# HKUDS/GPT-ST

Measured on AMD Instinct MI355X. Metric: pretrain steps/sec at (B=32,T=12,N=170,C=64), higher is better.
Workload: dtype f32; 1 GPU; BASELINE configs[1]: PEMS08-shape synthetic pretrain step, per-GPU B=32 T=12 N=170 C=64 base=1, epoch 200/300 (adaptive mask + KL), fwd+loss+bwd+clip+Adam, hipGraph=True, 4 full optimiser steps on 4 different resident batches per graph replay; global_batch=32, parallelism=dp1

## Files before the change

### gpt-st_amd/csrc/apply.hip

```cpp
#include "mfma_tile.h"
#include "wgrad64.h"
#include "kl_guest.h"
#ifdef GPTST_DEBUG
__device__ long long g_ap_ts[64];
static thread_local int g_ap_dbg = 0;
extern "C" int gptst_ap_dbg(int v) { g_ap_dbg = v; return 0; }
extern "C" int gptst_ap_ts(long long* out) { return (int)hipMemcpyFromSymbol(out, HIP_SYMBOL(g_ap_ts), sizeof(long long) * 64); }
#else
static constexpr int g_ap_dbg = 0;
#endif
thread_local int g_apply_tpw = 0;
thread_local int g_apply128_minwg = 768;
thread_local int g_apply128_v1 = 0;

template <int C, int PRO, int EPI>
__global__ __launch_bounds__(256) void apply_kernel(const float* __restrict__ A, const float* __restrict__ A2,
                                                    const float* __restrict__ W, long w_gstride, int transw,
                                                    const float* __restrict__ bias, const float* __restrict__ resid,
                                                    const float* __restrict__ resid2, float* __restrict__ out, float* __restrict__ colsum, RowMap rm, int dbg) {
    using T = Tile<C>;
    int tsi = 0;
#ifdef GPTST_DEBUG
#define TS() do { if (dbg && blockIdx.x == 100 && blockIdx.y == 0 && threadIdx.x == 0) g_ap_ts[tsi] = clock64(); ++tsi; } while (0)
#else
// ... 183 lines not shown
#pragma unroll
        for (int ct = 0; ct < 4; ++ct) acc[ct] = (f32x4){0.f, 0.f, 0.f, 0.f};
#pragma unroll
        for (int q = 0; q < 4; ++q) {
            const float av[4] = {a[q].x, a[q].y, a[q].z, a[q].w};
#pragma unroll
            for (int e = 0; e < 4; ++e) {
                acc[0] = __builtin_amdgcn_mfma_f32_16x16x4f32(av[e], bv[q][e].x, acc[0], 0, 0, 0);
                acc[1] = __builtin_amdgcn_mfma_f32_16x16x4f32(av[e], bv[q][e].y, acc[1], 0, 0, 0);
                acc[2] = __builtin_amdgcn_mfma_f32_16x16x4f32(av[e], bv[q][e].z, acc[2], 0, 0, 0);
                acc[3] = __builtin_amdgcn_mfma_f32_16x16x4f32(av[e], bv[q][e].w, acc[3], 0, 0, 0);
            }
        }
        SB();
#pragma unroll
        for (int r = 0; r < 4; ++r) {
            if (t * 16 + kk * 4 + r < rm.M) {
                float4 y = f4add(make_float4(acc[0][r], acc[1][r], acc[2][r], acc[3][r]), bias4);
                if (EPI == EPI_RES_LRELU) {
                    y = f4add(y, rv[r]);
                    y.x = lrelu(y.x); y.y = lrelu(y.y); y.z = lrelu(y.z); y.w = lrelu(y.w);
                }
                if (EPI == EPI_LRELU) { y.x = lrelu(y.x); y.y = lrelu(y.y); y.z = lrelu(y.z); y.w = lrelu(y.w); }
                if (EPI == EPI_ADD_DPRE) {
                    const float4 d = rv[r], o = rv2[r];
                    y.x = fmaf(d.x, lrelu_grad_from_out(o.x), y.x); y.y = fmaf(d.y, lrelu_grad_from_out(o.y), y.y);
                    y.z = fmaf(d.z, lrelu_grad_from_out(o.z), y.z); y.w = fmaf(d.w, lrelu_grad_from_out(o.w), y.w);
                }
                st4(out + orow[r], y);
            }
        }
    }
    if (colsum != nullptr) {
#pragma unroll
        for (int q = 0; q < 4; ++q) {
            cs[q].x = group_sum<16>(cs[q].x); cs[q].y = group_sum<16>(cs[q].y);
            cs[q].z = group_sum<16>(cs[q].z); cs[q].w = group_sum<16>(cs[q].w);
            if (j == 0) st4(&csl[wave][16 * q + 4 * kk], cs[q]);
        }
        __syncthreads();
        if (wave == 0) colsum[((size_t)blockIdx.y * rm.G + g) * C + lane] = (csl[0][lane] + csl[1][lane]) + (csl[2][lane] + csl[3][lane]);
    }
}

static void apply64_geometry(const RowMap& rm, bool has_colsum, int& tpw, int& gy) {
    const int ntiles = (rm.M + 15) / 16;
    long tot = (long)rm.G * ntiles;
    tpw = (int)((tot + 4 * 512 - 1) / (4 * 512));
    if (tpw > 2) tpw = 2;
    if (has_colsum && rm.G == 1) { const int lim = (ntiles + 4 * 128 - 1) / (4 * 128); if (tpw < lim) tpw = lim; }
    if (g_apply_tpw > 0) tpw = g_apply_tpw;
    if (tpw < 1) tpw = 1;
    gy = (ntiles + 4 * tpw - 1) / (4 * tpw);
}

template <int PRO, int EPI>
static void launch_apply64_t(const float* A, const float* A2, const float* W, long gs, int transw, const float* bias, const float* resid,
                             const float* resid2, float* out, float* colsum, RowMap rm, hipStream_t st) {
    int tpw, gy;
    apply64_geometry(rm, colsum != nullptr, tpw, gy);
    hipLaunchKernelGGL((apply64_kernel<PRO, EPI>), dim3(rm.G, gy), dim3(256), 0, st, A, A2, W, gs, transw, bias, resid, resid2, out, colsum, rm, tpw);
}

static int launch_apply64(const float* A, const float* A2, const float* W, long gs, int transw, const float* bias, const float* resid,
                          const float* resid2, float* out, float* colsum, RowMap rm, int pro, int epi, hipStream_t st) {
    if (pro == PRO_NONE && epi == EPI_PLAIN) launch_apply64_t<PRO_NONE, EPI_PLAIN>(A, A2, W, gs, transw, bias, resid, resid2, out, colsum, rm, st);
    else if (pro == PRO_NONE && epi == EPI_RES_LRELU) launch_apply64_t<PRO_NONE, EPI_RES_LRELU>(A, A2, W, gs, transw, bias, resid, resid2, out, colsum, rm, st);
    else if (pro == PRO_DPRE && epi == EPI_PLAIN) launch_apply64_t<PRO_DPRE, EPI_PLAIN>(A, A2, W, gs, transw, bias, resid, resid2, out, colsum, rm, st);
    else if (pro == PRO_NONE && epi == EPI_ADD_DPRE) launch_apply64_t<PRO_NONE, EPI_ADD_DPRE>(A, A2, W, gs, transw, bias, resid, resid2, out, colsum, rm, st);
    else if (pro == PRO_NONE && epi == EPI_LRELU) launch_apply64_t<PRO_NONE, EPI_LRELU>(A, A2, W, gs, transw, bias, resid, resid2, out, colsum, rm, st);
    else return GPTST_EARG;
    GPTST_CHECK_LAUNCH();
    return GPTST_OK;
}

template <int PRO, int U>
__global__ __launch_bounds__(256, 2) void wgrad64_kernel(const float* __restrict__ A, const float* __restrict__ D,
                                                         const float* __restrict__ D2, float* __restrict__ dW, RowMap rm,
                                                         int rows_per_split, int ostride, int csa) {
    __shared__ __attribute__((aligned(16))) float smem[WGRAD64_SMEM_FLOATS];
    wgrad64_body<PRO, U>(A, D, D2, dW, rm, rows_per_split, ostride, csa, blockIdx.x, blockIdx.y, smem);
}

template <int KIND, int CHAIN>
__global__ __launch_bounds__(256, 2) void applywg64_kernel(const float* __restrict__ dOut, const float* __restrict__ Y,
                                                            const float* __restrict__ S, const float* __restrict__ W, long w_gstride,
                                                            const float* __restrict__ resid, const float* __restrict__ resid2,
                                                            float* __restrict__ dS, float* __restrict__ dW, float* __restrict__ colsum,
                                                            RowMap rm, int tiles_per_wave) {
    __shared__ __attribute__((aligned(16))) float lds[APPLYWG64_LDS_FLOATS];
    applywg64_body<KIND, CHAIN>(dOut, Y, S, W, w_gstride, resid, resid2, dS, dW, colsum, rm, tiles_per_wave, blockIdx.x, blockIdx.y, lds);
}

GPTST_INTERNAL int gptst_apply_wgrad_geometry(int mode, int BT, int N, int* tpw) {
    RowMap rm = make_rowmap(mode, BT, N);
    int gy;
    apply64_geometry(rm, false, *tpw, gy);
    return gy;
}

extern "C" int gptst_apply_wgrad_nsplit(int mode, int BT, int N) {
    RowMap rm = make_rowmap(mode, BT, N);
    int tpw, gy;
    apply64_geometry(rm, false, tpw, gy);
    return gy;
}

extern "C" int gptst_apply_wgrad(const float* dOut, const float* Y, const float* S, const float* W, float* dS, float* dW, float* colsum,
                                 int premul, int mode, int BT, int N, int C, void* stream) {
    if (!dOut || !S || !W || !dS || !dW || BT <= 0 || N <= 0 || mode < 0 || mode > 1 || (Y && premul)) return GPTST_EARG;
    if (C != 64) return GPTST_ESHAPE;
    RowMap rm = make_rowmap(mode, BT, N);
    int tpw, gy;
    apply64_geometry(rm, false, tpw, gy);
    const dim3 grid(rm.G, gy);
    hipStream_t st = (hipStream_t)stream;
    if (Y) hipLaunchKernelGGL((applywg64_kernel<0, 0>), grid, dim3(256), 0, st, dOut, Y, S, W, (long)C * C, nullptr, nullptr, dS, dW, colsum, rm, tpw);
    else if (!premul) hipLaunchKernelGGL((applywg64_kernel<0, 1>), grid, dim3(256), 0, st, dOut, Y, S, W, (long)C * C, nullptr, nullptr, dS, dW, colsum, rm, tpw);
    else hipLaunchKernelGGL((applywg64_kernel<0, 2>), grid, dim3(256), 0, st, dOut, Y, S, W, (long)C * C, nullptr, nullptr, dS, dW, colsum, rm, tpw);
    GPTST_CHECK_LAUNCH();
    return GPTST_OK;
}

extern "C" int gptst_linear_bwd_nsplit(int rows) {
    RowMap rm = make_rowmap(2, rows, 1);
    int tpw, gy;
    apply64_geometry(rm, false, tpw, gy);
    return gy;
}

extern "C" int gptst_linear_bwd(const float* dY, const float* X, const float* Wp, const float* dOut, const float* out, float* dX, float* dWp,
                                float* dbp, int premul, int rows, int C, void* stream) {
    if (!dY || !X || !Wp || !dOut || !dX || !dWp || !dbp || rows <= 0 || (out && premul)) return GPTST_EARG;
    if (C != 64) return GPTST_ESHAPE;
    RowMap rm = make_rowmap(2, rows, 1);
    int tpw, gy;
    apply64_geometry(rm, false, tpw, gy);
    hipStream_t st = (hipStream_t)stream;
    if (out) hipLaunchKernelGGL((applywg64_kernel<1, 0>), dim3(1, gy), dim3(256), 0, st, dY, nullptr, X, Wp, 0L, dOut, out, dX, dWp, dbp, rm, tpw);
    else if (!premul) hipLaunchKernelGGL((applywg64_kernel<1, 1>), dim3(1, gy), dim3(256), 0, st, dY, nullptr, X, Wp, 0L, dOut, nullptr, dX, dWp, dbp, rm, tpw);
    else hipLaunchKernelGGL((applywg64_kernel<1, 2>), dim3(1, gy), dim3(256), 0, st, dY, nullptr, X, Wp, 0L, dOut, X, dX, dWp, dbp, rm, tpw);
    GPTST_CHECK_LAUNCH();
    return GPTST_OK;
}

template <int C, int PRO>
__global__ __launch_bounds__(256) void wgrad_kernel(const float* __restrict__ A, const float* __restrict__ D,
                                                    const float* __restrict__ D2, float* __restrict__ dW,
                                                    RowMap rm, int rows_per_split) {
    constexpr int NCT = C / 32;
    constexpr int TPW = NCT * NCT / 4;
    const int lane = threadIdx.x & 63, wave = threadIdx.x >> 6;
    const int j = lane & 31, h = lane >> 5;
    const int g = blockIdx.x, sp = blockIdx.y;
    const int mbeg = sp * rows_per_split;
    const int mend = min(rm.M, mbeg + rows_per_split);
    const int it = (wave * TPW) / NCT;
    f32x16 acc[TPW];
#pragma unroll
    for (int u = 0; u < TPW; ++u)
#pragma unroll
        for (int r = 0; r < 16; ++r) acc[u][r] = 0.f;

    for (int m = mbeg + h; m < mend + h; m += 2) {
        float a = 0.f;
        float d[TPW];
#pragma unroll
        for (int u = 0; u < TPW; ++u) d[u] = 0.f;
        if (m < mend) {
            const size_t off = ((size_t)g * rm.rs_g + (size_t)m * rm.rs_m) * C;
            a = A[off + it * 32 + j];
#pragma unroll
            for (int u = 0; u < TPW; ++u) {
                const int jt = (wave * TPW + u) % NCT;
                float dv = D[off + jt * 32 + j];
                if (PRO == PRO_DPRE) dv *= lrelu_grad_from_out(D2[off + jt * 32 + j]);
                d[u] = dv;
            }
        }
#pragma unroll
        for (int u = 0; u < TPW; ++u) acc[u] = __builtin_amdgcn_mfma_f32_32x32x2f32(a, d[u], acc[u], 0, 0, 0);
    }
    float* o = dW + ((size_t)sp * rm.G + g) * C * C;
#pragma unroll
    for (int u = 0; u < TPW; ++u) {
        const int jt = (wave * TPW + u) % NCT;
#pragma unroll
        for (int r = 0; r < 16; ++r) {
            const int row = (r & 3) + 8 * (r >> 2) + 4 * h;
            o[(size_t)(it * 32 + row) * C + jt * 32 + j] = acc[u][r];
        }
    }
}

#define AP128_NW 8
template <int PRO, int EPI, bool CS>
__global__ __launch_bounds__(64 * AP128_NW, 4) void apply128_kernel(const float* __restrict__ A, const float* __restrict__ A2,
                                                                    const float* __restrict__ W, long w_gstride, int transw,
                                                                    const float* __restrict__ bias, const float* __restrict__ resid,
                                                                    const float* __restrict__ resid2, float* __restrict__ out,
                                                                    float* __restrict__ colsum, RowMap rm, int tiles_per_wave) {
    constexpr int C = 128, Q = C / 16;
    extern __shared__ __attribute__((aligned(16))) float smem[];
    float* Wl = smem;
    float* csl = smem + C * C;
    const int lane = threadIdx.x & 63, wave = threadIdx.x >> 6;
    const int j = lane & 15, kk = lane >> 4;
    const int g = blockIdx.x;
    const int ntiles = (rm.M + 15) / 16;
    const int t0 = (blockIdx.y * AP128_NW + wave) * tiles_per_wave, t1 = min(ntiles, t0 + tiles_per_wave);
    float4 bias0 = f4zero(), bias1 = f4zero();
    if (bias != nullptr) { bias0 = ld4(bias + (size_t)g * C + 4 * j); bias1 = ld4(bias + (size_t)g * C + 64 + 4 * j); }
    float4 a[Q], on[Q];
    auto fetch = [&](int t) {
        const int m = min(t * 16 + j, rm.M - 1);
        const size_t off = ((size_t)g * rm.rs_g + (size_t)m * rm.rs_m) * C + 4 * kk;
#pragma unroll
        for (int q = 0; q < Q; ++q) {
            a[q] = ld4(A + off + 16 * q);
            if (PRO == PRO_DPRE) on[q] = ld4(A2 + off + 16 * q);
        }
    };
    if (t0 < t1) fetch(t0);
    load_w_lds<C, 64 * AP128_NW>(Wl, W + (size_t)g * w_gstride, transw, threadIdx.x);
// ... 346 lines not shown
```

### gpt-st_amd/csrc/guidein.hip

```cpp
#include "mfma_tile.h"
#include "kl_guest.h"

#define GI_CHUNKS 3

template <int C>
__global__ __launch_bounds__(256) void guide_in_fwd_kernel(const float* __restrict__ src, int lda, const float* __restrict__ w1,
                                                           const float* __restrict__ b1, const float* __restrict__ Wn, const float* __restrict__ bn,
                                                           float* __restrict__ h1, int BT, int N) {
    constexpr int LPR = C / 4, RPP = 256 / LPR, NQ = 256 / C, U = 4;
    __shared__ __attribute__((aligned(16))) float part[NQ * 2 * C];
    __shared__ __attribute__((aligned(16))) float vec[2 * C];
    const int n = blockIdx.x, chunk = blockIdx.y, tid = threadIdx.x;
    {
        const int q = tid / C, o = tid % C;
        const float* W = Wn + (size_t)n * C * C;
        float au = 0.f, ac = 0.f;
#pragma unroll 8
        for (int i = q * (C / NQ); i < (q + 1) * (C / NQ); ++i) {
            const float x = W[(size_t)i * C + o];
            au = fmaf(w1[i], x, au);
            ac = fmaf(b1[i], x, ac);
        }
        part[(q * 2 + 0) * C + o] = au;
        part[(q * 2 + 1) * C + o] = ac;
// ... 2 lines not shown
    if (tid < C) {
        float s0 = 0.f, s1 = 0.f;
#pragma unroll
        for (int q = 0; q < NQ; ++q) { s0 += part[(q * 2 + 0) * C + tid]; s1 += part[(q * 2 + 1) * C + tid]; }
        vec[tid] = s0; vec[C + tid] = s1 + bn[(size_t)n * C + tid];
    }
    __syncthreads();
    const int slot = tid / LPR, c4 = tid % LPR;
    const float4 u4 = ld4(vec + 4 * c4), k4 = ld4(vec + C + 4 * c4);
    const int per = (BT + GI_CHUNKS - 1) / GI_CHUNKS, r0 = chunk * per, r1 = min(BT, r0 + per);
    for (int rr = r0 + slot; rr < r1; rr += RPP * U) {
        float s[U];
#pragma unroll
        for (int u = 0; u < U; ++u) s[u] = src[((size_t)min(rr + u * RPP, r1 - 1) * N + n) * lda];
#pragma unroll
        for (int u = 0; u < U; ++u) {
            const int r = rr + u * RPP;
            if (r < r1) {
                float4 y = f4fma(s[u], u4, k4);
                y.x = lrelu(y.x); y.y = lrelu(y.y); y.z = lrelu(y.z); y.w = lrelu(y.w);
                st4(h1 + ((size_t)r * N + n) * C + 4 * c4, y);
            }
        }
    }
}

template <int C>
__global__ __launch_bounds__(256) void guide_in_bwd_kernel(const float* __restrict__ dPre, const float* __restrict__ src, int lda,
                                                           const float* __restrict__ w1, const float* __restrict__ b1, const float* __restrict__ Wn,
                                                           float* __restrict__ dWb, float* __restrict__ dinp, int BT, int N) {
    __shared__ __attribute__((aligned(16))) float lds[guide_in_bwd_lds_floats<C>()];
    guide_in_bwd_body<C>(dPre, src, lda, w1, b1, Wn, dWb, dinp, BT, N, blockIdx.x, lds);
}

extern "C" int gptst_guide_in_fwd(const float* src, int lda, const float* w1, const float* b1, const float* Wn, const float* bn, float* h1,
                                  int BT, int N, int C, void* stream) {
    if (!src || !w1 || !b1 || !Wn || !bn || !h1 || BT <= 0 || N <= 0 || lda <= 0) return GPTST_EARG;
    if (C == 64) hipLaunchKernelGGL((guide_in_fwd_kernel<64>), dim3(N, GI_CHUNKS), dim3(256), 0, (hipStream_t)stream, src, lda, w1, b1, Wn, bn, h1, BT, N);
    else if (C == 128) hipLaunchKernelGGL((guide_in_fwd_kernel<128>), dim3(N, GI_CHUNKS), dim3(256), 0, (hipStream_t)stream, src, lda, w1, b1, Wn, bn, h1, BT, N);
    else return GPTST_ESHAPE;
    GPTST_CHECK_LAUNCH();
    return GPTST_OK;
}

extern "C" int gptst_guide_in_bwd(const float* dPre, const float* src, int lda, const float* w1, const float* b1, const float* Wn, float* dWb,
                                  float* dinp, int BT, int N, int C, void* stream) {
    if (!dPre || !src || !w1 || !b1 || !Wn || !dWb || !dinp || BT <= 0 || N <= 0 || lda <= 0) return GPTST_EARG;
    if (C == 64) hipLaunchKernelGGL((guide_in_bwd_kernel<64>), dim3(N), dim3(256), 0, (hipStream_t)stream, dPre, src, lda, w1, b1, Wn, dWb, dinp, BT, N);
    else if (C == 128) hipLaunchKernelGGL((guide_in_bwd_kernel<128>), dim3(N), dim3(256), 0, (hipStream_t)stream, dPre, src, lda, w1, b1, Wn, dWb, dinp, BT, N);
    else return GPTST_ESHAPE;
    GPTST_CHECK_LAUNCH();
    return GPTST_OK;
}

template <int C>
__global__ __launch_bounds__(256) void guide_uc_kernel(const float* __restrict__ w1, const float* __restrict__ b1, const float* __restrict__ Wn,
                                                       const float* __restrict__ bn, float* __restrict__ uc) {
    constexpr int NQ = 256 / C;
    __shared__ __attribute__((aligned(16))) float part[NQ * 2 * C];
    const int n = blockIdx.x, tid = threadIdx.x;
    const int q = tid / C, o = tid % C;
    const float* W = Wn + (size_t)n * C * C;
    float au = 0.f, ac = 0.f;
#pragma unroll 8
    for (int i = q * (C / NQ); i < (q + 1) * (C / NQ); ++i) {
        const float x = W[(size_t)i * C + o];
        au = fmaf(w1[i], x, au);
        ac = fmaf(b1[i], x, ac);
    }
    part[(q * 2 + 0) * C + o] = au;
    part[(q * 2 + 1) * C + o] = ac;
    __syncthreads();
    if (tid < C) {
        float s0 = 0.f, s1 = 0.f;
#pragma unroll
        for (int qq = 0; qq < NQ; ++qq) { s0 += part[(qq * 2 + 0) * C + tid]; s1 += part[(qq * 2 + 1) * C + tid]; }
        uc[(size_t)n * 2 * C + tid] = s0;
        uc[(size_t)n * 2 * C + C + tid] = s1 + bn[(size_t)n * C + tid];
    }
}

#define GH_P 68
extern thread_local int g_apply_tpw;
__global__ __launch_bounds__(256, 2) void guide_head_fwd_kernel(const float* __restrict__ src, int lda, const float* __restrict__ uc,
                                                                const float* __restrict__ Wbt, const float* __restrict__ bbt,
                                                                const float* __restrict__ W3, const float* __restrict__ b3,
                                                                float* __restrict__ h1, float* __restrict__ h2, float* __restrict__ prob,
                                                                int* __restrict__ label, int N, int J, int tiles_per_wave) {
    constexpr int C = 64;
    __shared__ __attribute__((aligned(16))) float Wl[C * C];
    __shared__ __attribute__((aligned(16))) float tl[4][16 * GH_P];
    const int lane = threadIdx.x & 63, wave = threadIdx.x >> 6;
    const int j = lane & 15, kk = lane >> 4;
    const int g = blockIdx.x;
    const int ntiles = (N + 15) / 16;
    const int t0 = (blockIdx.y * 4 + wave) * tiles_per_wave, t1 = min(ntiles, t0 + tiles_per_wave);
    const float4 bias4 = ld4(bbt + (size_t)g * C + 4 * j);
    float4 bw[4];
#pragma unroll
    for (int q = 0; q < 4; ++q) bw[q] = j < J ? ld4(W3 + (size_t)j * C + 16 * q + 4 * kk) : f4zero();
    const float bj = j < J ? b3[j] : 0.f;
    float sn;
    float4 un[4], cn[4];
    auto fetch = [&](int t) {
        const int m = min(t * 16 + j, N - 1);
        sn = src[((size_t)g * N + m) * lda];
#pragma unroll
        for (int q = 0; q < 4; ++q) { un[q] = ld4(uc + (size_t)m * 2 * C + 16 * q + 4 * kk); cn[q] = ld4(uc + (size_t)m * 2 * C + C + 16 * q + 4 * kk); }
    };
    if (t0 < t1) fetch(t0);
    load_w_lds<C, 256>(Wl, Wbt + (size_t)g * C * C, 0, threadIdx.x);
    __syncthreads();
    float4 bv[4][4];
#pragma unroll
    for (int q = 0; q < 4; ++q)
#pragma unroll
        for (int e = 0; e < 4; ++e) bv[q][e] = ld4(Wl + (16 * q + 4 * kk + e) * C + 4 * j);
    float* tile = tl[wave];
    for (int t = t0; t < t1; ++t) {
        float4 a[4];
        const int mrow = t * 16 + j;
#pragma unroll
        for (int q = 0; q < 4; ++q) {
            float4 y = f4fma(sn, un[q], cn[q]);
            y.x = lrelu(y.x); y.y = lrelu(y.y); y.z = lrelu(y.z); y.w = lrelu(y.w);
            if (mrow < N) st4(h1 + ((size_t)g * N + mrow) * C + 16 * q + 4 * kk, y); else y = f4zero();
            a[q] = y;
        }
        if (t + 1 < t1) fetch(t + 1);
        SB();
        f32x4 acc[4];
#pragma unroll
        for (int ct = 0; ct < 4; ++ct) acc[ct] = (f32x4){0.f, 0.f, 0.f, 0.f};
#pragma unroll
        for (int q = 0; q < 4; ++q) {
            const float av[4] = {a[q].x, a[q].y, a[q].z, a[q].w};
#pragma unroll
            for (int e = 0; e < 4; ++e) {
                acc[0] = __builtin_amdgcn_mfma_f32_16x16x4f32(av[e], bv[q][e].x, acc[0], 0, 0, 0);
                acc[1] = __builtin_amdgcn_mfma_f32_16x16x4f32(av[e], bv[q][e].y, acc[1], 0, 0, 0);
                acc[2] = __builtin_amdgcn_mfma_f32_16x16x4f32(av[e], bv[q][e].z, acc[2], 0, 0, 0);
                acc[3] = __builtin_amdgcn_mfma_f32_16x16x4f32(av[e], bv[q][e].w, acc[3], 0, 0, 0);
            }
        }
        SB();
#pragma unroll
        for (int r = 0; r < 4; ++r) {
            const int m = t * 16 + kk * 4 + r;
            float4 y = f4add(make_float4(acc[0][r], acc[1][r], acc[2][r], acc[3][r]), bias4);
            y.x = lrelu(y.x); y.y = lrelu(y.y); y.z = lrelu(y.z); y.w = lrelu(y.w);
            if (m < N) st4(h2 + ((size_t)g * N + m) * C + 4 * j, y);
            st4(tile + (kk * 4 + r) * GH_P + 4 * j, y);
        }
        f32x4 z0 = {0.f, 0.f, 0.f, 0.f}, z1 = {0.f, 0.f, 0.f, 0.f};
#pragma unroll
        for (int q = 0; q < 4; ++q) {
            const float4 x = ld4(tile + j * GH_P + 16 * q + 4 * kk);
            z0 = __builtin_amdgcn_mfma_f32_16x16x4f32(x.x, bw[q].x, z0, 0, 0, 0);
            z1 = __builtin_amdgcn_mfma_f32_16x16x4f32(x.y, bw[q].y, z1, 0, 0, 0);
            z0 = __builtin_amdgcn_mfma_f32_16x16x4f32(x.z, bw[q].z, z0, 0, 0, 0);
            z1 = __builtin_amdgcn_mfma_f32_16x16x4f32(x.w, bw[q].w, z1, 0, 0, 0);
        }
#pragma unroll
        for (int r = 0; r < 4; ++r) {
            const int m = t * 16 + kk * 4 + r;
            const size_t i = (size_t)g * N + m;
            float v = z0[r] + z1[r] + bj;
            const float mx = group_max<16>(j < J ? v : -3.0e38f);
            const float e = j < J ? expf(v - mx) : 0.f;
            v = e / group_sum<16>(e);
            if (m < N && j < J) prob[i * J + j] = v;
            const float vv = j < J ? v : -3.0e38f;
            const float gm = group_max<16>(vv);
            const int first = (int)(-group_max<16>(vv == gm ? -(float)j : -3.0e38f));
            if (m < N && j == 0) label[i] = first;
        }
    }
}

extern "C" int gptst_guide_uc_floats(int N, int C) { return N * 2 * C; }

extern "C" int gptst_guide_head_fwd(const float* src, int lda, const float* w1, const float* b1, const float* Wn, const float* bn, const float* Wbt,
                                    const float* bbt, const float* W3, const float* b3, float* uc, float* h1, float* h2, float* prob, int* label,
                                    int BT, int N, int C, int J, void* stream) {
    if (!src || !w1 || !b1 || !Wn || !bn || !Wbt || !bbt || !W3 || !b3 || !uc || !h1 || !h2 || !prob || !label || BT <= 0 || N <= 0 || lda <= 0 || J <= 0)
        return GPTST_EARG;
    if (C != 64 || J > 16) return GPTST_ESHAPE;
    hipLaunchKernelGGL((guide_uc_kernel<64>), dim3(N), dim3(256), 0, (hipStream_t)stream, w1, b1, Wn, bn, uc);
    const int ntiles = (N + 15) / 16;
    int tpw = 1;
    if (g_apply_tpw > 0) tpw = g_apply_tpw;
    if (tpw < 1) tpw = 1;
    const int gy = (ntiles + 4 * tpw - 1) / (4 * tpw);
    hipLaunchKernelGGL(guide_head_fwd_kernel, dim3(BT, gy), dim3(256), 0, (hipStream_t)stream, src, lda, uc, Wbt, bbt, W3, b3, h1, h2, prob, label, N, J, tpw);
    GPTST_CHECK_LAUNCH();
    return GPTST_OK;
}
```

### gpt-st_amd/csrc/hypertem.hip

```cpp
#include "mfma_tile.h"
#include "wgrad64.h"
#include "kl_guest.h"
GPTST_STAMP_TABLES(hypertem)
GPTST_HANDOFF_COUNTER(hypertem)

#define HT_T 12
#ifndef HT_OCC
#define HT_OCC 2
#endif
#ifdef GPTST_DEBUG
__device__ long long g_ht_ts[64];
static thread_local int g_ht_dbg = 0, g_ht_nt_override = 0;
extern "C" int gptst_ht_dbg(int v) { g_ht_dbg = v; return 0; }
extern "C" int gptst_ht_variant(int fwd, int bwd) { g_ht_nt_override = fwd; (void)bwd; return 0; }
extern "C" int gptst_ht_ts(long long* out) { return (int)hipMemcpyFromSymbol(out, HIP_SYMBOL(g_ht_ts), sizeof(long long) * 64); }
#define HT_DBG(d) (d)
#else
#define HT_DBG(d) 0
static constexpr int g_ht_dbg = 0, g_ht_nt_override = 0;
#endif

__device__ __forceinline__ bool ht_work_at(int L, int ntiles, int B, int& b, int& tile) {
    const int xcd = L & 7, slot = L >> 3;
    b = xcd + 8 * (slot / ntiles);
    tile = slot % ntiles;
    return b < B;
}
__device__ __forceinline__ bool ht_work(int ntiles, int B, int& b, int& tile) { return ht_work_at(blockIdx.x, ntiles, B, b, tile); }

static int ht_pick_nt(int B, int N) {
    if (g_ht_nt_override >= 4 && g_ht_nt_override <= 16) return g_ht_nt_override;
    (void)B; (void)N;
    return 16;
}

__global__ __launch_bounds__(256, HT_OCC) void hypertem_fwd_kernel(const float* __restrict__ X, const float* __restrict__ G,
                                                              const float* __restrict__ Wbt, const float* __restrict__ bbt,
                                                              float* __restrict__ R_out, float* __restrict__ out, int N, int B, int NT,
                                                              int dbg) {
    constexpr int C = 64, P = C + 4, GP = 145;
    int tsi = 0;
#ifdef GPTST_DEBUG
#define TS() do { if ((dbg & 1) && blockIdx.x == 59 && threadIdx.x == 0) g_ht_ts[tsi] = clock64(); ++tsi; } while (0)
#else
#define TS() __builtin_amdgcn_sched_barrier(0)
#endif
    TS();
    extern __shared__ __attribute__((aligned(16))) float smem[];
    float* Xs = smem;
    float* Gs = Xs + HT_T * NT * P;
    int b, tile;
    if (!ht_work((N + NT - 1) / NT, B, b, tile)) return;
    const int n0 = tile * NT;
    const int tid = threadIdx.x, lane = tid & 63, wave = tid >> 6;
    {
        const int nl = tid >> 4, c4 = tid & 15;
        const int n = min(n0 + nl, N - 1);
        float4 v[HT_T];
        float gv[9];
#pragma unroll
        for (int t = 0; t < HT_T; ++t) v[t] = ld4(X + (((size_t)b * HT_T + t) * N + n) * C + 4 * c4);
#pragma unroll
        for (int k = 0; k < 9; ++k) gv[k] = G[min(n0 * 144 + tid + k * 256, N * 144 - 1)];
        if (nl < NT) {
#pragma unroll
            for (int t = 0; t < HT_T; ++t) st4(Xs + (t * NT + nl) * P + 4 * c4, n0 + nl < N ? v[t] : f4zero());
        }
#pragma unroll
        for (int k = 0; k < 9; ++k) {
            const int i = tid + k * 256;
            if (i < NT * 144) Gs[(i / 144) * GP + i % 144] = (n0 + i / 144 < N) ? gv[k] : 0.f;
        }
    }
    __syncthreads();
    TS();
    const int j = lane & 15, kk = lane >> 4;
    const int ja = j < NT ? j : 0;
    float4 bv[C / 16][4];
    float4 b4;
#define HT_LOAD_W(tt) do {                                                                                         \
        const float* W_ = Wbt + ((size_t)b * HT_T + (tt)) * C * C;                                                 \
        _Pragma("unroll") for (int q = 0; q < C / 16; ++q)                                                         \
            _Pragma("unroll") for (int e = 0; e < 4; ++e) bv[q][e] = ld4(W_ + (size_t)(16 * q + 4 * kk + e) * C + 4 * j); \
        b4 = ld4(bbt + ((size_t)b * HT_T + (tt)) * C + 4 * j);                                                     \
    } while (0)
    HT_LOAD_W(wave);
    for (int t = wave; t < HT_T; t += 4) {
        const size_t g = (size_t)b * HT_T + t;
        TS();
        float4 a4[C / 16];
#pragma unroll
        for (int q = 0; q < C / 16; ++q) a4[q] = f4zero();
        {
            const float* gr = Gs + ja * GP + t * HT_T;
            const float* xr = Xs + ja * P + 4 * kk;
#pragma unroll
            for (int u = 0; u < HT_T; ++u) {
                const float gu = gr[u];
#pragma unroll
                for (int q = 0; q < C / 16; ++q) a4[q] = f4fma(gu, ld4(xr + u * NT * P + 16 * q), a4[q]);
            }
        }
        TS();
        f32x4 acc[C / 16];
#pragma unroll
        for (int ct = 0; ct < C / 16; ++ct) acc[ct] = (f32x4){0.f, 0.f, 0.f, 0.f};
#pragma unroll
        for (int q = 0; q < C / 16; ++q) {
            const float av[4] = {a4[q].x, a4[q].y, a4[q].z, a4[q].w};
#pragma unroll
            for (int e = 0; e < 4; ++e) {
                acc[0] = __builtin_amdgcn_mfma_f32_16x16x4f32(av[e], bv[q][e].x, acc[0], 0, 0, 0);
                acc[1] = __builtin_amdgcn_mfma_f32_16x16x4f32(av[e], bv[q][e].y, acc[1], 0, 0, 0);
                acc[2] = __builtin_amdgcn_mfma_f32_16x16x4f32(av[e], bv[q][e].z, acc[2], 0, 0, 0);
                acc[3] = __builtin_amdgcn_mfma_f32_16x16x4f32(av[e], bv[q][e].w, acc[3], 0, 0, 0);
            }
        }
        TS();
        const float4 bias = b4;
        if (t + 4 < HT_T) HT_LOAD_W(t + 4);
        TS();
        if (R_out != nullptr && j < NT && n0 + j < N) {
#pragma unroll
            for (int q = 0; q < C / 16; ++q) st4_far(R_out + (g * N + n0 + j) * C + 16 * q + 4 * kk, a4[q]);
        }
#pragma unroll
        for (int r = 0; r < 4; ++r) {
            const int nl = kk * 4 + r;
            if (nl < NT && n0 + nl < N) {
                float4 y = f4add(f4add(make_float4(acc[0][r], acc[1][r], acc[2][r], acc[3][r]), bias), ld4(Xs + (t * NT + nl) * P + 4 * j));
                y.x = lrelu(y.x); y.y = lrelu(y.y); y.z = lrelu(y.z); y.w = lrelu(y.w);
                st4(out + (g * N + n0 + nl) * C + 4 * j, y);
            }
        }
        TS();
    }
}

static size_t ht_smem(int NT) { return ((size_t)HT_T * NT * 68 + NT * 145) * sizeof(float); }

extern "C" int gptst_hypertem_fwd(const float* X, const float* G, const float* Wbt, const float* bbt, float* R_out, float* out, int B,
                                  int T, int N, int C, void* stream) {
    if (!X || !G || !Wbt || !bbt || !out || T != HT_T) return GPTST_EARG;
    if (C != 64) return GPTST_ESHAPE;
    static int done = 0;
    if (!done) { hipFuncSetAttribute((const void*)hypertem_fwd_kernel, hipFuncAttributeMaxDynamicSharedMemorySize, (int)ht_smem(16)); done = 1; }
    const int NT = ht_pick_nt(B, N);
    hipLaunchKernelGGL(hypertem_fwd_kernel, dim3(8 * ((B + 7) / 8) * ((N + NT - 1) / NT)), dim3(256), ht_smem(NT), (hipStream_t)stream, X, G, Wbt, bbt, R_out, out, N, B, NT, g_ht_dbg);
    GPTST_CHECK_LAUNCH();
    return GPTST_OK;
}

template <bool HASY, bool PREMUL, int PAIR>
__device__ __forceinline__ void hypertem_bwd_stage(const float* __restrict__ dOut, const float* __restrict__ Y,
                                                   const float* __restrict__ X, const float* __restrict__ G,
                                                   const float* __restrict__ Wbt, float* __restrict__ dX,
                                                   float* __restrict__ dbias, float* __restrict__ dG, int N, int B, int dbg, int b, int tile,
                                                   float* __restrict__ smem, float4 (&dp)[HT_T]) {
    constexpr int C = 64, P = C + 4, GP = 145, NT = 16;
    float* Ds = smem;
    float* Gs = Ds + HT_T * NT * P;
    const int n0 = tile * NT;
    const int tid = threadIdx.x, lane = tid & 63, wave = tid >> 6;
    const int nl = tid >> 4, c4 = tid & 15;
    const bool valid = n0 + nl < N;
    const size_t rowoff = ((size_t)b * HT_T * N + min(n0 + nl, N - 1)) * C + 4 * c4;
    const int j = lane & 15, kk = lane >> 4;
    float4 aq[C / 16][C / 16];
#define HT_LOAD_WT(tt) do {                                                                                         \
        const float* W_ = Wbt + ((size_t)b * HT_T + (tt)) * C * C;                                                  \
        _Pragma("unroll") for (int it = 0; it < C / 16; ++it)                                                       \
            _Pragma("unroll") for (int q = 0; q < C / 16; ++q) aq[it][q] = ld4(W_ + (size_t)(it * 16 + j) * C + 16 * q + 4 * kk); \
    } while (0)
    static_assert(!(HASY && PREMUL), "one sign operand per launch");
    const float* __restrict__ Sg = HASY ? Y : X;
    float4 yv[HT_T];
    float gv[9];
    unsigned sb0 = 0u, sb1 = 0u;
#pragma unroll
    for (int t = 0; t < 4; ++t) { if (PAIR != 2) dp[t] = ld4(dOut + rowoff + (size_t)t * N * C); if (HASY || PREMUL) yv[t] = ld4(Sg + rowoff + (size_t)t * N * C); }
#pragma unroll
    for (int k = 0; k < 9; ++k) gv[k] = G[min(n0 * 144 + tid + k * 256, N * 144 - 1)];
    HT_LOAD_WT(wave);
#pragma unroll
    for (int t = 4; t < HT_T; ++t) { if (PAIR != 2) dp[t] = ld4(dOut + rowoff + (size_t)t * N * C); if (HASY || PREMUL) yv[t] = ld4(Sg + rowoff + (size_t)t * N * C); }
    SB();
#pragma unroll
    for (int grp = 0; grp < HT_T / 4; ++grp) {
#pragma unroll
        for (int tt = 0; tt < 4; ++tt) {
            const int t = 4 * grp + tt;
            float4 v = dp[t];
            if (HASY) v = make_float4(dp[t].x * lrelu_grad_from_out(yv[t].x), dp[t].y * lrelu_grad_from_out(yv[t].y),
                                      dp[t].z * lrelu_grad_from_out(yv[t].z), dp[t].w * lrelu_grad_from_out(yv[t].w));
            if (PREMUL) {
                const unsigned m4 = (yv[t].x > 0.f ? 1u : 0u) | (yv[t].y > 0.f ? 2u : 0u) | (yv[t].z > 0.f ? 4u : 0u) | (yv[t].w > 0.f ? 8u : 0u);
                if (t < 8) sb0 |= m4 << (4 * t); else sb1 |= m4 << (4 * (t - 8));
            }
            if (!valid) v = f4zero();
            dp[t] = v;
            st4(Ds + (t * NT + nl) * P + 4 * c4, v);
        }
        if (grp == 0) {
#pragma unroll
            for (int k = 0; k < 9; ++k) {
                const int i = tid + k * 256;
                Gs[(i / 144) * GP + i % 144] = (n0 + i / 144 < N) ? gv[k] : 0.f;
            }
        }
        __syncthreads();
        SB();
        if (PAIR != 0 && grp == 0) GPTST_STAMP(PAIR == 2 ? 6 : 1);
        const int t = 4 * grp + wave;
        if (HT_DBG(dbg) & 32) continue;
        const size_t g = (size_t)b * HT_T + t;
        float* dt = Ds + t * NT * P;
        float s = 0.f;
        if (dbias != nullptr) {
#pragma unroll
            for (int r = 0; r < NT; ++r) s += dt[r * P + lane];
        }
        float4 bq[C / 16];
#pragma unroll
        for (int q = 0; q < C / 16; ++q) bq[q] = ld4(dt + j * P + 16 * q + 4 * kk);
        f32x4 acc[C / 16];
#pragma unroll
        for (int it = 0; it < C / 16; ++it) acc[it] = (f32x4){0.f, 0.f, 0.f, 0.f};
        if (!(HT_DBG(dbg) & 64))
#pragma unroll
        for (int q = 0; q < C / 16; ++q) {
#pragma unroll
// ... 483 lines not shown
                const float4 bias = b4;
                if (t + NW < HT_T) HTC_LOAD_W(S.Wbt, S.bbt, t + NW);
                SB();
                if (S.R_out != nullptr && n0 + j < N) {
#pragma unroll
                    for (int q = 0; q < C / 16; ++q) st4_far(S.R_out + (g * N + n0 + j) * C + 16 * q + 4 * kk, a4[q]);
                }
#pragma unroll
                for (int r = 0; r < 4; ++r) {
                    const int nl = kk * 4 + r;
                    if (n0 + nl < N) {
                        float4 y = f4add(f4add(make_float4(acc[0][r], acc[1][r], acc[2][r], acc[3][r]), bias), ld4(Xs + (t * NT + nl) * P + 4 * j));
                        y.x = lrelu(y.x); y.y = lrelu(y.y); y.z = lrelu(y.z); y.w = lrelu(y.w);
                        st4(S.out + (g * N + n0 + nl) * C + 4 * j, y);
                    }
                }
            }
        }
    }
#undef HTC_LOAD_G
#undef HTC_STORE_G
#undef HTC_LOAD_W
}

static int ht_chain_args(HtChain& ch, const float* X, int nstage, const void* Gs, const void* Wbts, const void* bbts, const void* Rs, const void* outs,
                         int B, int T, int N, int C) {
    if (!X || nstage < 1 || nstage > 3 || !Gs || !Wbts || !bbts || !Rs || !outs || T != HT_T || B <= 0 || N <= 0) return GPTST_EARG;
    if (C != 64) return GPTST_ESHAPE;
    ch.nstage = nstage; ch.X = X;
    for (int s = 0; s < 3; ++s) {
        const int k = s < nstage ? s : nstage - 1;
        ch.st[s] = HtStage{((const float* const*)Gs)[k], ((const float* const*)Wbts)[k], ((const float* const*)bbts)[k],
                           ((float* const*)Rs)[k], ((float* const*)outs)[k]};
        if (!ch.st[s].G || !ch.st[s].Wbt || !ch.st[s].bbt || !ch.st[s].out) return GPTST_EARG;
    }
    return GPTST_OK;
}

static int ht_chain_grid(int B, int N) { return 8 * ((B + 7) / 8) * ((N + 15) / 16); }

extern "C" int gptst_hypertem_chain_fwd(const float* X, int nstage, const void* Gs, const void* Wbts, const void* bbts, const void* Rs,
                                        const void* outs, int B, int T, int N, int C, void* stream) {
    HtChain ch;
    const int rc = ht_chain_args(ch, X, nstage, Gs, Wbts, bbts, Rs, outs, B, T, N, C);
    if (rc != GPTST_OK) return rc;
    const dim3 grid(ht_chain_grid(B, N));
    const int smem = (int)ht_smem(16);
    hipStream_t st = (hipStream_t)stream;
    const KlGuest none{};
#define HTC_LAUNCH(NS_) do {                                                                                                          \
        static int done_ = 0;                                                                                                          \
        if (!done_) { (void)hipFuncSetAttribute((const void*)hypertem_chain_fwd_kernel<NS_, 0>, hipFuncAttributeMaxDynamicSharedMemorySize, smem); done_ = 1; } \
        hipLaunchKernelGGL((hypertem_chain_fwd_kernel<NS_, 0>), grid, dim3(64 * HTC_NW), smem, st, ch, N, B, none);                          \
    } while (0)
    if (nstage == 1) HTC_LAUNCH(1); else if (nstage == 2) HTC_LAUNCH(2); else HTC_LAUNCH(3);
#undef HTC_LAUNCH
    GPTST_CHECK_LAUNCH();
    return GPTST_OK;
}

GPTST_INTERNAL int gptst_tail_geometry(int rows, int* rows_per_block);
GPTST_INTERNAL int gptst_apply_wgrad_geometry(int mode, int BT, int N, int* tpw);

extern "C" int gptst_kl_guest_blocks(int stage, int B, int T, int N) {
    if (B <= 0 || T <= 0 || N <= 0) return GPTST_EARG;
    int aux;
    if (stage == 1) return gptst_tail_geometry(B * T * N, &aux);
    if (stage == 2) return B * T * gptst_apply_wgrad_geometry(0, B * T, N, &aux);
    if (stage == 3) return N;
    return GPTST_EARG;
}

extern "C" int gptst_hypertem_chain_fwd_kl(const float* X, int nstage, const void* Gs, const void* Wbts, const void* bbts, const void* Rs,
                                           const void* outs, int B, int T, int N, int C, int stage, const void* ops, int v0, int v1, int HS,
                                           int lda, float w, void* stream) {
    HtChain ch;
    const int rc = ht_chain_args(ch, X, nstage, Gs, Wbts, bbts, Rs, outs, B, T, N, C);
    if (rc != GPTST_OK) return rc;
    if (!ops || stage < 1 || stage > 3) return GPTST_EARG;
    if (nstage != 2 || HTC_NW != 4 || HS <= 0 || HS > TL_MAXJ) return GPTST_ESHAPE;
    const int nv = gptst_kl_guest_blocks(stage, B, T, N);
    if (v0 < 0 || v1 <= v0 || v1 > nv) return GPTST_EARG;
    const float* const* p = (const float* const*)ops;
    const int np = stage == 1 ? 7 : stage == 2 ? 6 : 7;
    for (int i = 0; i < np; ++i) if (!p[i]) return GPTST_EARG;
    KlGuest kg{};
    kg.base = ht_chain_grid(B, N);
    kg.v0 = v0;
    if (stage == 1) {
        TailArgs& t = kg.tail;
        t.X = p[0]; t.W = p[1]; t.prob = p[2]; t.c = p[3]; t.dX = (float*)p[4]; t.part = (float*)p[5]; t.sws = (float*)p[6];
        t.rows = B * T * N; t.J = HS; t.N = N; t.w = w; t.premul = 1;
        gptst_tail_geometry(t.rows, &t.rows_per_block);
    } else if (stage == 2) {
        kg.dOut = p[0]; kg.S = p[1]; kg.W = p[2]; kg.dS = (float*)p[3]; kg.dW = (float*)p[4]; kg.colsum = (float*)p[5];
        kg.rm = make_rowmap(0, B * T, N);
        gptst_apply_wgrad_geometry(0, B * T, N, &kg.tpw);
    } else {
        if (lda <= 0) return GPTST_EARG;
        kg.dPre = p[0]; kg.src = p[1]; kg.lda = lda; kg.w1 = p[2]; kg.b1 = p[3]; kg.Wn = p[4]; kg.dWb = (float*)p[5]; kg.dinp = (float*)p[6];
        kg.BT = B * T; kg.N = N;
    }
    const dim3 grid(kg.base + (v1 - v0));
    const size_t sg = kl_guest_lds_bytes(stage), sh = ht_smem(16);
    const int smem = (int)(sg > sh ? sg : sh);
    hipStream_t st = (hipStream_t)stream;
#define HTC_LAUNCH(G_) do {                                                                                                           \
        static int done_ = 0;                                                                                                          \
        if (!done_) { (void)hipFuncSetAttribute((const void*)hypertem_chain_fwd_kernel<2, G_>, hipFuncAttributeMaxDynamicSharedMemorySize, smem); done_ = 1; } \
        hipLaunchKernelGGL((hypertem_chain_fwd_kernel<2, G_>), grid, dim3(64 * HTC_NW), smem, st, ch, N, B, kg);                           \
    } while (0)
    if (stage == 1) HTC_LAUNCH(1); else if (stage == 2) HTC_LAUNCH(2); else HTC_LAUNCH(3);
#undef HTC_LAUNCH
    GPTST_CHECK_LAUNCH();
    return GPTST_OK;
}
```

### gpt-st_amd/csrc/kl_guest.h

```cpp
#pragma once
#include "mfma_tile.h"
#include "wgrad64.h"

#define TL_MAXJ 16

struct TailArgs {
    const float* X; const float* W; const float* b; float* dX; float* part; float* sws;
    int rows, J, rows_per_block;
    const float* src; const float* mask; float* out; int lda; float sigma, mu, thresh;
    const float* prob; const float* c; int N; float w;
    int premul;
};

template <int C>
constexpr int tail_mfma_lds_floats() { return 4 * (16 * C + 16) + 4 * 16 * 17 + 8; }

template <int KIND, int C>
__device__ __forceinline__ void tail_mfma_body(const TailArgs& t, int blk, float* __restrict__ lds) {
    constexpr int Q = C / 16, HF = C / 64;
    float (*fold)[16 * C + 16] = reinterpret_cast<float (*)[16 * C + 16]>(lds);
    float (*at)[16][17] = reinterpret_cast<float (*)[16][17]>(lds + 4 * (16 * C + 16));
    float (*reds)[4] = reinterpret_cast<float (*)[4]>(lds + 4 * (16 * C + 16) + 4 * 16 * 17);
    const int J = t.J;
    const int lane = threadIdx.x & 63, wave = threadIdx.x >> 6;
// ... 60 lines not shown
                        a[r] = (d > 0.f ? 1.f : (d < 0.f ? -1.f : 0.f)) * M * t.sigma;
                    }
                    t.out[e] = o;
                }
            }
        } else {
#pragma unroll
            for (int r = 0; r < 4; ++r) {
                const size_t i = tb + 4 * kk + r;
                const bool ok = i < r1 && j < J;
                float e_ = 0.f, p_ = 1.f;
                if (ok) { e_ = o0[r]; p_ = o1[r]; }
                const float se = group_sum<16>(e_);
                if (ok && e_ > 0.f) s0 += e_ * (logf(e_) - logf(p_));
                a[r] = ok ? t.w * (p_ * se - e_) : 0.f;
            }
        }
#pragma unroll
        for (int r = 0; r < 4; ++r) {
            gb += a[r];
#pragma unroll
            for (int hf = 0; hf < HF; ++hf) {
                gw[hf][0] = __builtin_amdgcn_mfma_f32_16x16x4f32(a[r], xd[hf][r].x, gw[hf][0], 0, 0, 0);
                gw[hf][1] = __builtin_amdgcn_mfma_f32_16x16x4f32(a[r], xd[hf][r].y, gw[hf][1], 0, 0, 0);
                gw[hf][2] = __builtin_amdgcn_mfma_f32_16x16x4f32(a[r], xd[hf][r].z, gw[hf][2], 0, 0, 0);
                gw[hf][3] = __builtin_amdgcn_mfma_f32_16x16x4f32(a[r], xd[hf][r].w, gw[hf][3], 0, 0, 0);
            }
        }
#pragma unroll
        for (int r = 0; r < 4; ++r) at[wave][4 * kk + r][j] = a[r];
        f32x4 dx[HF][4];
#pragma unroll
        for (int hf = 0; hf < HF; ++hf)
#pragma unroll
            for (int ct = 0; ct < 4; ++ct) dx[hf][ct] = (f32x4){0.f, 0.f, 0.f, 0.f};
#pragma unroll
        for (int s = 0; s < 4; ++s) {
            if (s < nks) {
                const float as = at[wave][j][4 * s + kk];
#pragma unroll
                for (int hf = 0; hf < HF; ++hf) {
                    dx[hf][0] = __builtin_amdgcn_mfma_f32_16x16x4f32(as, bd[hf][s].x, dx[hf][0], 0, 0, 0);
                    dx[hf][1] = __builtin_amdgcn_mfma_f32_16x16x4f32(as, bd[hf][s].y, dx[hf][1], 0, 0, 0);
                    dx[hf][2] = __builtin_amdgcn_mfma_f32_16x16x4f32(as, bd[hf][s].z, dx[hf][2], 0, 0, 0);
                    dx[hf][3] = __builtin_amdgcn_mfma_f32_16x16x4f32(as, bd[hf][s].w, dx[hf][3], 0, 0, 0);
                }
            }
        }
#pragma unroll
        for (int r = 0; r < 4; ++r) {
            const size_t i = tb + 4 * kk + r;
#pragma unroll
            for (int hf = 0; hf < HF; ++hf) {
                float4 v = make_float4(dx[hf][0][r], dx[hf][1][r], dx[hf][2][r], dx[hf][3][r]);
                if (t.premul) {
                    v.x *= lrelu_grad_from_out(xd[hf][r].x); v.y *= lrelu_grad_from_out(xd[hf][r].y);
                    v.z *= lrelu_grad_from_out(xd[hf][r].z); v.w *= lrelu_grad_from_out(xd[hf][r].w);
                }
                if (i < r1) st4(t.dX + i * C + 64 * hf + 4 * j, v);
            }
        }
    }
#pragma unroll
    for (int r = 0; r < 4; ++r)
#pragma unroll
        for (int hf = 0; hf < HF; ++hf) st4(&fold[wave][(4 * kk + r) * C + 64 * hf + 4 * j], make_float4(gw[hf][0][r], gw[hf][1][r], gw[hf][2][r], gw[hf][3][r]));
    gb += __shfl_xor(gb, 16, 64); gb += __shfl_xor(gb, 32, 64);
    if (kk == 0) fold[wave][16 * C + j] = gb;
    s0 = group_sum<64>(s0); s1 = group_sum<64>(s1);
    if (lane == 0) { reds[0][wave] = s0; reds[1][wave] = s1; }
    __syncthreads();
    float* mine = t.part + (size_t)blk * (J * C + J);
    for (int o = threadIdx.x; o < J * C; o += 256) mine[o] = (fold[0][o] + fold[1][o]) + (fold[2][o] + fold[3][o]);
    if ((int)threadIdx.x < J) mine[J * C + threadIdx.x] = (fold[0][16 * C + threadIdx.x] + fold[1][16 * C + threadIdx.x]) + (fold[2][16 * C + threadIdx.x] + fold[3][16 * C + threadIdx.x]);
    if (threadIdx.x == 0) {
        float* w = t.sws + 4 * (size_t)blk;
        const float v0 = (reds[0][0] + reds[0][1]) + (reds[0][2] + reds[0][3]), v1 = (reds[1][0] + reds[1][1]) + (reds[1][2] + reds[1][3]);
        if (KIND == 0) { w[0] = v0; w[1] = v1; } else { w[2] = v0; }
    }
}

constexpr int APPLYWG64_LDS_FLOATS = 4 * 64 * 64 + 4 * 64;

template <int KIND, int CHAIN>
__device__ __forceinline__ void applywg64_body(const float* __restrict__ dOut, const float* __restrict__ Y, const float* __restrict__ S,
                                               const float* __restrict__ W, long w_gstride, const float* __restrict__ resid,
                                               const float* __restrict__ resid2, float* __restrict__ dS, float* __restrict__ dW,
                                               float* __restrict__ colsum, RowMap rm, int tiles_per_wave, int g, int split, float* __restrict__ lds) {
    constexpr int C = 64, TP = C + 4;
    float* smem = lds;
    float (*csl)[C] = reinterpret_cast<float (*)[C]>(lds + 4 * C * C);
    float* Wl = smem;
    const int lane = threadIdx.x & 63, wave = threadIdx.x >> 6;
    float* tile = smem + C * C + wave * 16 * TP;
    const int j = lane & 15, kk = lane >> 4;
    const int ntiles = (rm.M + 15) / 16;
    const int t0 = (split * 4 + wave) * tiles_per_wave, t1 = min(ntiles, t0 + tiles_per_wave);
    float4 d[4], y[4], a[4];
    auto fetch = [&](int t) {
#pragma unroll
        for (int s4 = 0; s4 < 4; ++s4) {
            const int m = min(t * 16 + 4 * s4 + kk, rm.M - 1);
            const size_t off = ((size_t)g * rm.rs_g + (size_t)m * rm.rs_m) * C + 4 * j;
            d[s4] = ld4(dOut + off); a[s4] = ld4(S + off);
            if (KIND == 0 && CHAIN == 0) y[s4] = ld4(Y + off);
        }
    };
    if (t0 < t1) fetch(t0);
    load_w_lds<C, 256>(Wl, W + (size_t)g * w_gstride, KIND == 0 ? 1 : 0, threadIdx.x);
    __syncthreads();
    float4 bv[4][4];
#pragma unroll
    for (int q = 0; q < 4; ++q)
#pragma unroll
        for (int e = 0; e < 4; ++e) bv[q][e] = ld4(Wl + (16 * q + 4 * kk + e) * C + 4 * j);
    f32x4 accw[4][4];
#pragma unroll
    for (int ca = 0; ca < 4; ++ca)
#pragma unroll
        for (int cb = 0; cb < 4; ++cb) accw[ca][cb] = (f32x4){0.f, 0.f, 0.f, 0.f};
    float4 cs = f4zero();
    for (int t = t0; t < t1; ++t) {
        if (KIND == 1 && t != t0) fetch(t);
        SB();
#pragma unroll
        for (int s4 = 0; s4 < 4; ++s4) {
            float4 v = d[s4];
            if (KIND == 0 && CHAIN == 0) v = make_float4(d[s4].x * lrelu_grad_from_out(y[s4].x), d[s4].y * lrelu_grad_from_out(y[s4].y),
                                                         d[s4].z * lrelu_grad_from_out(y[s4].z), d[s4].w * lrelu_grad_from_out(y[s4].w));
            if (t * 16 + 4 * s4 + kk >= rm.M) v = f4zero();
            d[s4] = v;
            cs = f4add(cs, v);
            st4(tile + (4 * s4 + kk) * TP + 4 * j, v);
        }
#pragma unroll
        for (int s4 = 0; s4 < 4; ++s4) {
            const float sv[4] = {a[s4].x, a[s4].y, a[s4].z, a[s4].w}, dv[4] = {d[s4].x, d[s4].y, d[s4].z, d[s4].w};
#pragma unroll
            for (int ca = 0; ca < 4; ++ca)
#pragma unroll
                for (int cb = 0; cb < 4; ++cb)
                    accw[ca][cb] = __builtin_amdgcn_mfma_f32_16x16x4f32(KIND == 0 ? sv[ca] : dv[ca], KIND == 0 ? dv[cb] : sv[cb], accw[ca][cb], 0, 0, 0);
        }
        SB();
        float4 ap[4];
#pragma unroll
        for (int q = 0; q < 4; ++q) ap[q] = ld4(tile + j * TP + 16 * q + 4 * kk);
        const int tcur = t;
        if (KIND == 0 && t + 1 < t1) fetch(t + 1);
        float4 rv[4], rv2[4];
        if (KIND == 1 || CHAIN == 2) {
#pragma unroll
            for (int r = 0; r < 4; ++r) {
                const int m = min(tcur * 16 + kk * 4 + r, rm.M - 1);
                const size_t off = ((size_t)g * rm.rs_g + (size_t)m * rm.rs_m) * C + 4 * j;
                if (KIND == 1) rv[r] = ld4(resid + off);
                if (KIND == 1 && CHAIN != 1) rv2[r] = ld4(resid2 + off);
                if (KIND == 0 && CHAIN == 2) rv2[r] = ld4(S + off);
            }
        }
        SB();
        f32x4 acc[4];
#pragma unroll
        for (int ct = 0; ct < 4; ++ct) acc[ct] = (f32x4){0.f, 0.f, 0.f, 0.f};
#pragma unroll
        for (int q = 0; q < 4; ++q) {
            const float av[4] = {ap[q].x, ap[q].y, ap[q].z, ap[q].w};
#pragma unroll
            for (int e = 0; e < 4; ++e) {
                acc[0] = __builtin_amdgcn_mfma_f32_16x16x4f32(av[e], bv[q][e].x, acc[0], 0, 0, 0);
                acc[1] = __builtin_amdgcn_mfma_f32_16x16x4f32(av[e], bv[q][e].y, acc[1], 0, 0, 0);
                acc[2] = __builtin_amdgcn_mfma_f32_16x16x4f32(av[e], bv[q][e].z, acc[2], 0, 0, 0);
                acc[3] = __builtin_amdgcn_mfma_f32_16x16x4f32(av[e], bv[q][e].w, acc[3], 0, 0, 0);
            }
        }
        SB();
#pragma unroll
        for (int r = 0; r < 4; ++r) {
            const int m = tcur * 16 + kk * 4 + r;
            float4 o4 = make_float4(acc[0][r], acc[1][r], acc[2][r], acc[3][r]);
            if (KIND == 1 && CHAIN == 0) {
                o4.x = fmaf(rv[r].x, lrelu_grad_from_out(rv2[r].x), o4.x); o4.y = fmaf(rv[r].y, lrelu_grad_from_out(rv2[r].y), o4.y);
                o4.z = fmaf(rv[r].z, lrelu_grad_from_out(rv2[r].z), o4.z); o4.w = fmaf(rv[r].w, lrelu_grad_from_out(rv2[r].w), o4.w);
            }
            if (KIND == 1 && CHAIN != 0) o4 = f4add(o4, rv[r]);
            if (CHAIN == 2) {
                o4.x *= lrelu_grad_from_out(rv2[r].x); o4.y *= lrelu_grad_from_out(rv2[r].y);
                o4.z *= lrelu_grad_from_out(rv2[r].z); o4.w *= lrelu_grad_from_out(rv2[r].w);
            }
            if (m < rm.M) st4(dS + ((size_t)g * rm.rs_g + (size_t)m * rm.rs_m) * C + 4 * j, o4);
        }
    }
    cs.x += __shfl_xor(cs.x, 16, 64); cs.y += __shfl_xor(cs.y, 16, 64); cs.z += __shfl_xor(cs.z, 16, 64); cs.w += __shfl_xor(cs.w, 16, 64);
    cs.x += __shfl_xor(cs.x, 32, 64); cs.y += __shfl_xor(cs.y, 32, 64); cs.z += __shfl_xor(cs.z, 32, 64); cs.w += __shfl_xor(cs.w, 32, 64);
    if (kk == 0) st4(&csl[wave][4 * j], cs);
    __syncthreads();
    float* red = smem + wave * C * C;
#pragma unroll
    for (int ca = 0; ca < 4; ++ca)
#pragma unroll
        for (int r = 0; r < 4; ++r)
            st4(&red[(4 * (kk * 4 + r) + ca) * C + 4 * j], make_float4(accw[ca][0][r], accw[ca][1][r], accw[ca][2][r], accw[ca][3][r]));
    __syncthreads();
    if (colsum != nullptr && threadIdx.x < C)
        colsum[((size_t)split * rm.G + g) * C + threadIdx.x] = (csl[0][threadIdx.x] + csl[1][threadIdx.x]) + (csl[2][threadIdx.x] + csl[3][threadIdx.x]);
    float* o = dW + ((size_t)split * rm.G + g) * (size_t)(C * C);
#pragma unroll
    for (int k = 0; k < C * C / 4 / 256; ++k) {
        const int f = threadIdx.x + k * 256;
        const float4 s4 = f4add(f4add(ld4(smem + 4 * f), ld4(smem + C * C + 4 * f)), f4add(ld4(smem + 2 * C * C + 4 * f), ld4(smem + 3 * C * C + 4 * f)));
        st4(o + 4 * f, s4);
    }
}

template <int C>
constexpr int guide_in_bwd_lds_floats() { return (256 / (C / 4)) * 2 * C + 2 * C; }

template <int C>
__device__ __forceinline__ void guide_in_bwd_body(const float* __restrict__ dPre, const float* __restrict__ src, int lda,
                                                  const float* __restrict__ w1, const float* __restrict__ b1, const float* __restrict__ Wn,
                                                  float* __restrict__ dWb, float* __restrict__ dinp, int BT, int N, int n, float* __restrict__ lds) {
    constexpr int LPR = C / 4, RPP = 256 / LPR, U = 6, PP = 256 / C;
    float* red = lds;
    float* vec = lds + RPP * 2 * C;
    const int tid = threadIdx.x;
    const int slot = tid / LPR, c4 = tid % LPR;
    float4 P = f4zero(), Q = f4zero();
    for (int rr = slot; rr < BT; rr += RPP * U) {
        float4 d[U];
        float s[U];
#pragma unroll
        for (int u = 0; u < U; ++u) {
            const size_t r = (size_t)min(rr + u * RPP, BT - 1) * N + n;
            d[u] = ld4(dPre + r * C + 4 * c4);
            s[u] = src[r * lda];
        }
#pragma unroll
        for (int u = 0; u < U; ++u)
            if (rr + u * RPP < BT) { P = f4fma(s[u], d[u], P); Q = f4add(Q, d[u]); }
    }
    st4(red + (slot * 2 + 0) * C + 4 * c4, P); st4(red + (slot * 2 + 1) * C + 4 * c4, Q);
    __syncthreads();
    for (int i = tid; i < 2 * C; i += 256) {
        float s = 0.f;
#pragma unroll 4
        for (int sl = 0; sl < RPP; ++sl) s += red[(sl * 2 + i / C) * C + i % C];
        vec[i] = s;
    }
    __syncthreads();
    float* row = dWb + (size_t)n * (C * C + C);
    for (int f = tid; f < C * C / 4; f += 256) {
        const int i = f / LPR, o4 = f % LPR;
        const float wi = w1[i], bb = b1[i];
        const float4 p4 = ld4(vec + 4 * o4), q4 = ld4(vec + C + 4 * o4);
        st4(row + (size_t)i * C + 4 * o4, make_float4(fmaf(wi, p4.x, bb * q4.x), fmaf(wi, p4.y, bb * q4.y), fmaf(wi, p4.z, bb * q4.z), fmaf(wi, p4.w, bb * q4.w)));
    }
    if (tid < C) row[C * C + tid] = vec[C + tid];
    {
        const int i = tid / PP, pq = tid % PP;
        const float* Wr = Wn + (size_t)n * C * C + (size_t)i * C + pq * (C / PP);
        float r1 = 0.f, r2 = 0.f;
#pragma unroll
        for (int k = 0; k < C / PP / 4; ++k) {
            const float4 x = ld4(Wr + 4 * k);
            r1 += f4dot(x, ld4(vec + pq * (C / PP) + 4 * k));
            r2 += f4dot(x, ld4(vec + C + pq * (C / PP) + 4 * k));
        }
        r1 = group_sum<PP>(r1); r2 = group_sum<PP>(r2);
        if (pq == 0) { dinp[(size_t)n * 2 * C + i] = r1; dinp[(size_t)n * 2 * C + C + i] = r2; }
    }
}

struct KlGuest {
    int base;
    int v0;
    TailArgs tail;
    const float* dOut; const float* S; const float* W; float* dS; float* dW; float* colsum; RowMap rm; int tpw;
    const float* dPre; const float* src; int lda; const float* w1; const float* b1; const float* Wn; float* dWb; float* dinp; int BT, N;
};

template <int STAGE>
__device__ __forceinline__ void kl_guest_run(const KlGuest& k, int v, float* lds) {
    if constexpr (STAGE == 1) tail_mfma_body<1, 64>(k.tail, v, lds);
    else if constexpr (STAGE == 2) applywg64_body<0, 2>(k.dOut, nullptr, k.S, k.W, 64L * 64, nullptr, nullptr, k.dS, k.dW, k.colsum, k.rm, k.tpw,
                                                        v % k.rm.G, v / k.rm.G, lds);
    else guide_in_bwd_body<64>(k.dPre, k.src, k.lda, k.w1, k.b1, k.Wn, k.dWb, k.dinp, k.BT, k.N, v, lds);
}

inline size_t kl_guest_lds_bytes(int stage) {
    const int f = stage == 1 ? tail_mfma_lds_floats<64>() : stage == 2 ? APPLYWG64_LDS_FLOATS : guide_in_bwd_lds_floats<64>();
    return (size_t)f * sizeof(float);
}
```

### gpt-st_amd/engine.py

```python
import contextlib
import os
import threading
from typing import Any, NamedTuple

import torch

from . import _C, ops
from .ops import (EPI_ADD_DPRE, EPI_ADD_PREMUL, EPI_LRELU, EPI_PREMUL, EPI_PLAIN, EPI_RES_LRELU, MODE_NODE, MODE_SHARED, MODE_TIME, PRO_DPRE, PRO_NONE)

TF_NAMES = ("ln_day", "ln_week", "ln1", "ln2", "ln")


class ZeroArena:

    def __init__(self, device):
        self.device, self.buf, self.off, self.need = device, None, 0, 0

    def begin(self, zero=True):
        pending = None
        if self.buf is None or self.buf.numel() < self.need:
            self.buf = torch.zeros(max(self.need, 1), device=self.device) if self.need else None
        elif self.buf is not None:
            if zero:
                self.buf.zero_()
# ... 63 lines not shown
        if carry is not None and carry.jobs:
            self.jobs.jobs = carry.jobs + self.jobs.jobs
            carry.jobs = []

    def gram(self, A, dG, dA, N, nsG):
        self.grams.append((A, dG, dA, N, nsG))

    def timefeat(self, p, g, pfx, tidx, dout, spg=False):
        self.tf.append(_tf_job(p, pfx, tidx, spg)._replace(grads=_tf_tensors(g, pfx), dout=dout))

    def flush_async(self, tidx):
        if self.bucket_inline and self.on_bucket is not None and self.nbucket == 0 and (self.jobs.jobs or self.late.jobs or self.grams or self.tf):
            self._run(tidx)
            self.fork_side.wait_stream(torch.cuda.current_stream())
            with torch.cuda.stream(self.fork_side):
                self.on_bucket(0)
            self.forked = True
            self.nbucket += 1

    def flush(self, tidx):
        self._run(tidx)
        if self.forked:
            torch.cuda.current_stream().wait_stream(self.fork_side)
            self.forked = False

    def _run(self, tidx):
        gr, self.grams = sorted(self.grams, key=lambda t: t[0].data_ptr()), []
        while gr:
            A, dG, dA, N, nsG = gr.pop(0)
            while gr and gr[0][0].data_ptr() == A.data_ptr() + 4 * A.numel() and gr[0][1].data_ptr() == dG.data_ptr() + 4 * dG.numel() \
                    and gr[0][2].data_ptr() == dA.data_ptr() + 4 * dA.numel() and gr[0][3:] == (N, nsG):
                A2, dG2, dA2 = gr.pop(0)[:3]
                A = torch.as_strided(A, (A.shape[0] + A2.shape[0],) + tuple(A.shape[1:]), A.stride())
                dG = torch.as_strided(dG, (dG.shape[0] + dG2.shape[0],) + tuple(dG.shape[1:]), dG.stride())
                dA = torch.as_strided(dA, (dA.shape[0] + dA2.shape[0],) + tuple(dA.shape[1:]), dA.stride())
            ops.gram_bwd(A, dG, out=dA, layers=A.shape[0] // N, nsplit=nsG)
        self.jobs.jobs, self.late.jobs = self.jobs.jobs + self.late.jobs, []
        self.jobs.launch()
        tf, self.tf = self.tf, []
        ops.timefeat_jobs_bwd(tf, tidx)
        self.keep = []


def _zeros(ref, *shape):
    if CTX.ARENA is not None:
        return CTX.ARENA.zeros(*shape)
    return torch.zeros(*shape, device=ref.device)


def _tf_tensors(d, pfx):
    out = []
    for n in TF_NAMES:
        out += [d[pfx + n + ".weight"], d[pfx + n + ".bias"]]
    return out


def _tf_job(p, pfx, tidx, spg=False):
    B, T = tidx.shape[0], tidx.shape[1]
    rows, K = (B, T) if spg else (B * T, 1)
    return ops.TimefeatJob(_tf_tensors(p, pfx), rows, K)


DROP_R = os.environ.get("GPTST_DROP_R", "0") == "1"


class HtSaved(NamedTuple):
    x: Any
    R: Any
    out: Any
    G: Any
    Wbt: Any


class WgradParts(NamedTuple):
    dW: Any
    ns: int
    db: Any


def _ht_fused_bwd(dims):
    return dims[3] == 64 and FUSE_HT_BWD


def hypertem_core_fwd(x, G, Wbt, bbt, dims):
    B, T, N, C = dims
    if C == 64:
        keep = not (DROP_R and _ht_fused_bwd(dims) and ops.wgrad_nsplit(MODE_TIME, B * T, N, C) == 1)
        R, out = ops.hypertem_fwd(x.view(B, T, N, C), G, Wbt, bbt, want_R=keep)
        R, out = (R.view(-1, C) if keep else None), out.view(-1, C)
    else:
        R = ops.tmix(x.view(B, T, N, C), G).view(-1, C)
        out = ops.apply(R, Wbt, MODE_TIME, B * T, N, bias=bbt, resid=x, epi=EPI_RES_LRELU)
    return out, HtSaved(x, R, out, G, Wbt)


FUSE_HT_BWD = True


def graph_grad_splits(dims):
    return dims[0] if dims[3] == 64 else 1


CHAIN128 = os.environ.get("GPTST_CHAIN128", "1") == "1"


def chain_ok(dims):
    return _ht_fused_bwd(dims) or (CHAIN128 and dims[3] == 128)


def _wb_parts(dWb, C, ns=1):
    return WgradParts(dWb[:, :C * C], ns, dWb[:, C * C:])


def _wgrad_parts(a, dout, out, mode, dims):
    B, T, N, C = dims
    dWb, ns = ops.wgrad(a, dout, mode, B * T, N, D2=out, pro=PRO_NONE if out is None else PRO_DPRE, colsum_d=True)
    return _wb_parts(dWb, C, ns)


def _genlin_bwd(dout, out, x, W, mode, dims, chain, premul=False):
    B, T, N, C = dims
    BT = B * T
    if C == 64:
        dx, dW, db, ns = ops.apply_wgrad(dout, None if chain else out, x, W, mode, BT, N, premul=chain and premul)
        return dx, WgradParts(dW, ns, db)
    if chain:
        dx = (ops.apply(dout, W, mode, BT, N, transw=True, resid2=x, epi=EPI_PREMUL) if premul
              else ops.apply(dout, W, mode, BT, N, transw=True))
        return dx, _wgrad_parts(x, dout, None, mode, dims)
    dx = ops.apply(dout, W, mode, BT, N, A2=out, transw=True, pro=PRO_DPRE)
    return dx, _wgrad_parts(x, dout, out, mode, dims)


def hypertem_core_bwd(saved, dout, dG_out, dims, chain=False, premul=False):
    B, T, N, C = dims
    x, R, out, G, Wbt = saved
    BT = B * T
    v = lambda a: a.view(B, T, N, C)
    assert not chain or chain_ok(dims)
    if _ht_fused_bwd(dims):
        dx, dWb, ns, _ = ops.hypertem_bwd_wgrad(v(dout), None if chain else v(out), v(x), G, Wbt, v(R) if R is not None else None, dG=dG_out,
                                                premul=chain and premul)
        return dx.view(-1, C), _wb_parts(dWb, C, ns)
    hp = _wgrad_parts(R, dout, None if chain else out, MODE_TIME, dims)
    if C == 64:
        dx, _, _ = ops.hypertem_bwd(v(dout), v(out), v(x), G, Wbt, dG=dG_out, want_dbias=False)
    elif chain:
        dR = ops.apply(dout, Wbt, MODE_TIME, BT, N, transw=True)
        dx, _ = ops.tmix_bwd_chain(v(dR), v(x), G, v(dout), premul=premul, dG=dG_out[0])
    else:
        dR = ops.apply(dout, Wbt, MODE_TIME, BT, N, A2=out, transw=True, pro=PRO_DPRE)
        dx, _ = ops.tmix_bwd(v(dR), v(x), G, v(dout), v(out), dG=dG_out[0])
    return dx.view(-1, C), hp


CARRY_RED = os.environ.get("GPTST_CARRY_RED", "1") == "1"
CARRY_MB = float(os.environ.get("GPTST_CARRY_MB", "25"))
CARRY_KL = os.environ.get("GPTST_CARRY_KL", "1") == "1"
PAIR_UNDER_DP = os.environ.get("GPTST_PAIR_UNDER_DP", "1") == "1"
PAIR_BWD = os.environ.get("GPTST_PAIR_BWD", "1") == "1"


@contextlib.contextmanager
def no_handoffs():
    from . import _C
    keep = (CTX.NO_HANDOFFS, _C.lib().value("gptst_mask_cooperative_state"))
    CTX.NO_HANDOFFS = True
    _C.lib().call("gptst_mask_cooperative", 0)
    try:
        yield
    finally:
        CTX.NO_HANDOFFS = keep[0]
        _C.lib().call("gptst_mask_cooperative", keep[1])


def pair_bwd_on():
    return PAIR_BWD and not CTX.NO_HANDOFFS


def cross_role():
    return 0 if CTX.NO_HANDOFFS else CROSS_ROLE


def _ht_pair_shape_ok(dims):
    B, T, N, C = dims
    if T != 12 or C != 64:
        return False
    ns = ops.wgrad_nsplit(MODE_TIME, B * T, N, C)
    rps = (-(-N // ns) + 1) & ~1
    return -(-N // rps) == ns


def ht_pair_ok(saved1, saved0, dims):
    return (pair_bwd_on() and dims[3] == 64 and not isinstance(saved1, EncIn) and saved1.R is not None and saved0.R is not None
            and _ht_fused_bwd(dims) and _ht_pair_shape_ok(dims))


class PendingH1:

    def __init__(self, saved, dd, dG, dWb):
        self.saved, self.dd, self.dG, self.dWb = saved, dd, dG, dWb


def ht_pair_bwd(saved1, saved0, dout, dG1, dG0, dims, dWb1=None):
    B, T, N, C = dims
    if not ht_pair_ok(saved1, saved0, dims):
        assert dWb1 is None
        return None
    s1, s0 = saved1, saved0
    v = lambda a: a.view(B, T, N, C)
    r = ops.hypertem_bwd_pair(v(dout), v(s1.x), s1.G, s1.Wbt, v(s1.R), v(s0.x), s0.G, s0.Wbt, v(s0.R), dG1, dG0, _zeros(dout, B), dWb1=dWb1)
    assert r is not None or dWb1 is None
    if r is None:
        return None
    dmid, dx0, dWb1, dWb0, ns = r
    return dx0.view(-1, C), _wb_parts(dWb1, C, ns), _wb_parts(dWb0, C, ns)


FUSE_CROSS = os.environ.get("GPTST_FUSE_CROSS", "1") == "1"
CAP_LIN = os.environ.get("GPTST_CAP_LIN", "1") == "1"
CROSS_ROLE = int(os.environ.get("GPTST_CROSS_ROLE", "1"))


class CapSaved(NamedTuple):
    x: Any
    out: Any
    rec: Any
    c: Any
    s: Any
    v: Any
    Ht: Any
    Rt: Any
    dyn: Any
    Wn: Any
    Y: Any


class CapParts(NamedTuple):
    wn: WgradParts
    ddyn: Any
    dlogit: Any


def cap_head_fwd(p, pfx, x, dadj, dyn, dims, num_route, HS, HT):
    B, T, N, C = dims
    c, s, Y = ops.cap_route_fwd(x.view(B, T, N, C), p[pfx + "ln_p.weight"], p[pfx + "ln_p.bias"], dadj, HS, num_route,
                                reduce_nodes=CTX.NODE_REDUCE, want_Y=True)
    fused = ops.cap_cross_rec_fwd(s, dyn, p[pfx + "mask_template"], c, B, T, N, HS, HT) if (FUSE_CROSS and CTX.NODE_REDUCE is None) else None
    if fused is not None:
        v, Ht, Rt, rec = fused
    else:
        v, Ht, Rt = ops.cap_cross_fwd(s, dyn, p[pfx + "mask_template"], B, T, HS, HT)
        rec = ops.cap_rec_fwd(c, v, N, C)
    return rec, c, (s, v, Ht, Rt, Y)


def cap_core_fwd(p, pfx, x, dadj, dyn, Wn, bn, dims, num_route, HS, HT):
    B, T, N, C = dims
    rec, c, (s, v, Ht, Rt, Y) = cap_head_fwd(p, pfx, x, dadj, dyn, dims, num_route, HS, HT)
    out = ops.apply(rec, Wn, MODE_NODE, B * T, N, bias=bn, resid=x, epi=EPI_RES_LRELU)
    return out, c, CapSaved(x, out, rec, c, s, v, Ht, Rt, dyn, Wn, Y)


CHAIN_FWD = os.environ.get("GPTST_CHAIN_FWD", "1") == "1"


def chain_fwd_ok(dims):
    return CHAIN_FWD and dims[3] == 64 and not DROP_R


def ht_chain_fwd(x, stages, dims, kl=None):
    B, T, N, C = dims
    res = ops.hypertem_chain_fwd(x.view(B, T, N, C), stages, guest=kl.guest() if kl is not None else None)
    saved, xin = [], x
    for (G, Wbt, _b), (R, o) in zip(stages, res):
        o = o.view(-1, C)
        saved.append(HtSaved(xin, R.view(-1, C), o, G, Wbt))
        xin = o
    return saved, xin


def cap_core_bwd(p, g, pfx, saved, dout, dims, HS, HT, red, chain=False):
    B, T, N, C = dims
    x, out, rec, c, s, v, Ht, Rt, dyn, Wn, Y = saved
    BT, dev = B * T, x.device
    assert not chain or chain_ok(dims)
    drec, wn = _genlin_bwd(dout, out, rec, Wn, MODE_NODE, dims, chain)
    dc1, dv = ops.cap_rec_bwd(drec, c, v, reduce_nodes=CTX.NODE_REDUCE)
    gw, gb = g[pfx + "ln_p.weight"], g[pfx + "ln_p.bias"]
    if FUSE_CROSS and CAP_LIN and C == 64 and CTX.NODE_REDUCE is None and Y is None:
        carry = red.take_carry(CARRY_MB) if cross_role() and _C.lib().value("gptst_cap_route_roles_ok", B, T, N, C, HS, HT) == 1 else None
        lin = ops.cap_cross_route_lin_bwd(x.view(B, T, N, C), p[pfx + "ln_p.weight"], p[pfx + "ln_p.bias"], c, dc1, dv, s, Rt, Ht, dyn,
                                          p[pfx + "mask_template"], dout, None if chain else out, chain, B, T, HS, HT,
                                          flags=_zeros(x, 4 * B) if cross_role() else None, jobs=carry)
        red.untake(carry)
        if lin is not None:
            dx, dWp, dbp, dlogit, ddyn = lin
            red.jobs.bwd_pool(_ones(dev, dWp.shape[0]), dWp, gw.view(1, C * C))
            red.jobs.bwd_pool(_ones(dev, dbp.shape[0]), dbp, gb.view(1, C))
            return dx, CapParts(wn, ddyn, dlogit)
    fused = None
    if FUSE_CROSS and CTX.NODE_REDUCE is None and Y is None:
        fused = ops.cap_cross_route_bwd(x.view(B, T, N, C), p[pfx + "ln_p.weight"], p[pfx + "ln_p.bias"], c, dc1, dv, s, Rt, Ht, dyn,
                                        p[pfx + "mask_template"], B, T, HS, HT, flags=_zeros(x, 4 * B) if cross_role() else None)
    if fused is not None:
        dY, dlogit, ddyn = fused
    else:
        dS, ddyn = ops.cap_cross_bwd(dv, s, Rt, Ht, dyn, p[pfx + "mask_template"], B, T, HS, HT)
        dY, dlogit = ops.cap_route_bwd(x.view(B, T, N, C), p[pfx + "ln_p.weight"], p[pfx + "ln_p.bias"], c, dc1, dS, Y=Y)
    if C == 64:
        dx, dWp, dbp, ns2 = ops.linear_bwd(dY, x, p[pfx + "ln_p.weight"], dout, None if chain else out, premul=chain)
        red.jobs.bwd_pool(_ones(dev, ns2), dWp, gw.view(1, C * C))
        red.jobs.bwd_pool(_ones(dev, ns2), dbp, gb.view(1, C))
    else:
        if chain:
            dx = ops.apply(dY, p[pfx + "ln_p.weight"], MODE_SHARED, BT, N, resid=dout, resid2=x, epi=EPI_ADD_PREMUL)
        else:
            dx = ops.apply(dY, p[pfx + "ln_p.weight"], MODE_SHARED, BT, N, resid=dout, resid2=out, epi=EPI_ADD_DPRE)
        dWp, ns2 = ops.wgrad(dY, x, MODE_SHARED, BT, N, colsum_a=True)
        wp = _wb_parts(dWp, C, ns2)
        red.jobs.bwd_pool(_ones(dev, ns2), wp.dW, gw.view(1, C * C))
        red.jobs.bwd_pool(_ones(dev, ns2), wp.db, gb.view(1, C))
    return dx, CapParts(wn, ddyn, dlogit)


_ONES = {}


def _ones(dev, n=1):
    if (dev, n) not in _ONES:
        _ONES[(dev, n)] = torch.ones(n, 1, device=dev)
    return _ONES[(dev, n)]


class CondLinSaved(NamedTuple):
    x: Any
    out: Any
    W: Any


def condlin_fwd(x, Wg, bg, mode, dims):
    B, T, N, C = dims
    out = ops.apply(x, Wg, mode, B * T, N, bias=bg, epi=EPI_LRELU)
    return out, CondLinSaved(x, out, Wg)


def condlin_bwd(saved, dout, emb, wpool, bpool, g_wpool, g_bpool, d_emb, mode, dims, red, chain=False, premul=False, carried=None):
    C = dims[3]
    R, K = emb.shape
    assert not chain or chain_ok(dims)
    dx, w = carried if carried is not None else _genlin_bwd(dout, saved.out, saved.x, saved.W, mode, dims, chain, premul)
    ns, db = w.ns, w.db
    dW = w.dW if w.dW.dim() == 2 else w.dW.view(ns * R, C * C)
    red.jobs.bwd_pool(emb, dW, g_wpool.view(K, C * C), nsplit=ns)
    red.jobs.bwd_pool(emb, db, g_bpool, nsplit=ns)
    red.jobs.bwd_emb(dW, wpool.view(K, C * C), d_emb, nsplit=ns)
# ... 38 lines not shown
    c1: Any
    c2: Any
    emb: Any
    gen: SthcnGen
    slot: Any


class GenAll(NamedTuple):
    sthcn: Any
    guide: Any
    pending: Any


def _sthcn_gen_jobs(p, pfx, emb, jobs, A_all, dims, G_all, slot=None):
    B, T, N, C = dims
    time_eb, teb, tes = emb
    ne, nes = p[pfx + "node_embeddings"], p[pfx + "node_embeddings_spg"]
    hts, cps = _sthcn_names(pfx)
    adj0 = p[hts[0] + "adj"]
    d, Hm = adj0.shape[0], adj0.shape[1]
    cadj, tadj = p[cps[0] + "adj"], p[cps[0] + "t_adj"]
    ds, HS, HT = cadj.shape[0], cadj.shape[1], tadj.shape[1]
    for i, h in enumerate(hts):
        jobs.fwd(ne, p[h + "adj"].view(d, Hm * T), out=A_all[i])
        jobs.gram(ne, p[h + "adj"].view(d, Hm * T), out=G_all[i], A=A_all[i])
    Wb = [(jobs.fwd(time_eb, p[h + "weights_pool"]), jobs.fwd(time_eb, p[h + "bias_pool"])) for h in hts]
    Wn = [(jobs.fwd(nes, p[c + "weights_spa"]), jobs.fwd(nes, p[c + "bias_spa"])) for c in cps]
    dadj = [jobs.fwd(teb, p[c + "adj"].view(ds, HS * N)) for c in cps]
    dyn = [jobs.fwd(tes, p[c + "t_adj"].view(ds, HT * T * HS)).view(B, HT, T * HS) for c in cps]
    return SthcnGen(emb, A_all, G_all, Wb, Wn, dadj, dyn, hts, cps, d, Hm, ds, HS, HT, slot)


def gen_all(p, tidx, dims, which=(ENC, DEC), guide=True, defer=False):
    B, T, N, C = dims
    tfj = []
    for pfx in which:
        tfj += [_tf_job(p, pfx + "time_feature1.", tidx), _tf_job(p, pfx + "time_feature1_.", tidx),
                _tf_job(p, pfx + "time_feature2.", tidx, spg=True)]
    if guide:
        tfj.append(_tf_job(p, GUIDE_TF, tidx))
    embs = ops.timefeat_jobs_fwd(tfj, tidx)
    jobs = ops.PoolJobs()
    now = ops.PoolJobs() if defer else jobs
    sthcn, gd = {}, None
    L = 4 * len(which)
    if guide:
        gj = now
        m = "encoder.MLP_RL."
        t4m = embs[-1]
        gd = (t4m, gj.fwd(p["encoder.neb4mask"], p[m + "weights_pool_spa"]), gj.fwd(p["encoder.neb4mask"], p[m + "bias_pool_spa"]),
              gj.fwd(t4m, p[m + "weights_pool_tem"]), gj.fwd(t4m, p[m + "bias_pool_tem"]))
    if L:
        adj0 = p[which[0] + "hyperTem1.adj"]
        Hm = adj0.shape[1]
        A_all = torch.empty(L, N, Hm * T, device=tidx.device)
        G_all = torch.empty(L, N, T, T, device=tidx.device)
        for k, pfx in enumerate(which):
            sthcn[pfx] = _sthcn_gen_jobs(p, pfx, embs[3 * k:3 * k + 3], jobs, A_all[4 * k:4 * k + 4], dims, G_all[4 * k:4 * k + 4], (k, len(which)))
    now.launch()
    return GenAll(sthcn, gd, jobs if defer else None)


def sthcn_fwd(p, pfx, tidx, x, dims, num_route, gen=None, head=None, next_gen=None, kl=None):
    if gen is None:
        gen = gen_all(p, tidx, dims, which=(pfx,), guide=False).sthcn[pfx]
    ht = gen.ht
    cap = lambda i, x: cap_core_fwd(p, gen.cps[i], x, gen.dadj[i], gen.dyn[i], *gen.Wn[i], dims, num_route, gen.HS, gen.HT)
    pairs = chain_fwd_ok(dims)
    nhead = None
    x, h1 = head if head is not None else hypertem_core_fwd(x, *ht(0), dims)
    x, c1, sc1 = cap(0, x)
    if pairs:
        if kl is not None and kl.c1 is None:
            kl.c1 = c1
        (h2, h3), x = ht_chain_fwd(x, [ht(1), ht(2)], dims, kl)
    else:
        x, h2 = hypertem_core_fwd(x, *ht(1), dims)
        x, h3 = hypertem_core_fwd(x, *ht(2), dims)
    x, _, sc2 = cap(1, x)
    if pairs and next_gen is not None:
        (h4, h1n), xn = ht_chain_fwd(x, [ht(3), next_gen.ht(0)], dims, kl)
        x, nhead = h4.out, (xn, h1n)
    else:
        x, h4 = hypertem_core_fwd(x, *ht(3), dims)
    return x, c1, SthcnSaved(h1, h2, h3, h4, sc1, sc2, gen.emb, gen, gen.slot), nhead


def _grad_buffers(red, slot, N, T, HmT, ref, nsG):
    if slot is None:
        return torch.empty(4, nsG, N, T, T, device=ref.device), torch.empty(4, N, HmT, device=ref.device)
    k, n = slot
    if red._dG is None or red._dG.shape[0] != 4 * n:
        red._dG = torch.empty(4 * n, nsG, N, T, T, device=ref.device)
        red._dA = torch.empty(4 * n, N, HmT, device=ref.device)
    return red._dG[4 * k:4 * k + 4], red._dA[4 * k:4 * k + 4]


def sthcn_bwd(p, g, pfx, tidx, sv, dout, dims, red, chain=False, premul_in=False, defer_h1=False, after_pending=None):
    B, T, N, C = dims
    time_eb, teb, tes = sv.emb
    gn = sv.gen
    A_all, hts, cps, d, Hm, ds, HS, HT = gn.A_all, gn.hts, gn.cps, gn.d, gn.Hm, gn.ds, gn.HS, gn.HT
    ne, nes = p[pfx + "node_embeddings"], p[pfx + "node_embeddings_spg"]
    dne, dnes = g[pfx + "node_embeddings"], g[pfx + "node_embeddings_spg"]
    d_te, d_teb, d_tes = _zeros(time_eb, *time_eb.shape), _zeros(teb, *teb.shape), _zeros(tes, *tes.shape)
    nsG = graph_grad_splits(dims)
    dG_all, dA_all = _grad_buffers(red, sv.slot, N, T, Hm * T, dout, nsG)
    J = red.jobs
    CC, BT = C * C, B * T

    def queue_ht(h, hp):
        J.bwd_pool(time_eb, hp.dW, g[h + "weights_pool"].view(d, CC), nsplit=hp.ns)
        J.bwd_pool(time_eb, hp.db, g[h + "bias_pool"], nsplit=hp.ns)
        J.bwd_emb(hp.dW, p[h + "weights_pool"].view(d, CC), d_te, nsplit=hp.ns)
        J.bwd_emb(hp.db, p[h + "bias_pool"], d_te, nsplit=hp.ns)

    def queue_cap(c, cp):
        w, ns = cp.wn, cp.wn.ns
        dW2 = w.dW if w.dW.dim() == 2 else w.dW.view(ns * N, CC)
        J.bwd_pool(nes, dW2, g[c + "weights_spa"].view(d, CC), nsplit=ns)
        J.bwd_pool(nes, w.db, g[c + "bias_spa"], nsplit=ns)
        J.bwd_emb(dW2, p[c + "weights_spa"].view(d, CC), dnes, nsplit=ns)
        J.bwd_emb(w.db, p[c + "bias_spa"], dnes, nsplit=ns)
        dd2 = cp.ddyn.view(B, HT * T * HS)
        J.bwd_pool(tes, dd2, g[c + "t_adj"].view(ds, HT * T * HS))
        J.bwd_emb(dd2, p[c + "t_adj"].view(ds, HT * T * HS), d_tes)
        dl2 = cp.dlogit.view(BT, HS * N)
        J.bwd_pool(teb, dl2, g[c + "adj"].view(ds, HS * N))
        J.bwd_emb(dl2, p[c + "adj"].view(ds, HS * N), d_teb)

    if isinstance(dout, PendingH1):
        up = dout
        dd, _, hp4 = ht_pair_bwd(up.saved, sv.h4, up.dd, up.dG, dG_all[3], dims, dWb1=up.dWb)
        red.keep.append(up)
        if after_pending is not None:
            after_pending()
    else:
        dd, hp4 = hypertem_core_bwd(sv.h4, dout, dG_all[3], dims, chain, True)
    queue_ht(hts[3], hp4)
    dd, cp2 = cap_core_bwd(p, g, cps[1], sv.c2, dd, dims, HS, HT, red, chain)
    queue_cap(cps[1], cp2)
    pair = ht_pair_bwd(sv.h3, sv.h2, dd, dG_all[2], dG_all[1], dims) if chain and pair_bwd_on() else None
    if pair is not None:
        dd, hp3, hp2 = pair
    else:
        dd, hp3 = hypertem_core_bwd(sv.h3, dd, dG_all[2], dims, chain, True)
        dd, hp2 = hypertem_core_bwd(sv.h2, dd, dG_all[1], dims, chain, True)
    queue_ht(hts[2], hp3)
    queue_ht(hts[1], hp2)
    dd, cp1 = cap_core_bwd(p, g, cps[0], sv.c1, dd, dims, HS, HT, red, chain)
    queue_cap(cps[0], cp1)
    if isinstance(sv.h1, EncIn):
        assert chain
        e = sv.h1
        w, bi = p["encoder.dim_in_flow.weight"], p["encoder.dim_in_flow.bias"]
        if nsG == B:
            dWb, _, dinp = ops.encin_ht1_bwd(dd.view(B, T, N, C), e.source, e.mask, e.fill, w, bi, e.Wbt, e.ab, e.wv, dG=dG_all[0])
        else:
            dWb, dGb, dinp = ops.encin_ht1_bwd(dd.view(B, T, N, C), e.source, e.mask, e.fill, w, bi, e.Wbt, e.ab, e.wv)
            torch.sum(dGb, 0, out=dG_all[0][0])
        hp1 = _wb_parts(dWb, C)
        wb = _wb_view(g["encoder.dim_in_flow.weight"], g["encoder.dim_in_flow.bias"])
        if wb is not None:
            red.jobs.bwd_pool(_ones(dd.device, dinp.shape[0]), dinp, wb)
        else:
            g["encoder.dim_in_flow.weight"].add_(dinp[:, :C].sum(0).view(C, 1))
            g["encoder.dim_in_flow.bias"].add_(dinp[:, C:].sum(0))
        red.keep.append((dinp, dWb))
        dd = None
    elif defer_h1:
        assert chain and premul_in
        ns = ops.wgrad_nsplit(MODE_TIME, B * T, N, C)
        dWb = torch.empty(ns * B * T, C * C + C, device=dd.device, dtype=torch.float32)
        hp1 = _wb_parts(dWb, C, ns)
        dd = PendingH1(sv.h1, dd, dG_all[0], dWb)
    else:
        dd, hp1 = hypertem_core_bwd(sv.h1, dd, dG_all[0], dims, chain, premul_in)
    queue_ht(hts[0], hp1)
    red.gram(A_all.view(4 * N, Hm, T), dG_all, dA_all.view(4 * N, Hm, T), N, nsG)
    for i, h in enumerate(hts):
        red.late.bwd_pool(ne, dA_all[i], g[h + "adj"].view(d, Hm * T))
        red.late.bwd_emb(dA_all[i], p[h + "adj"].view(d, Hm * T), dne)
    red.timefeat(p, g, pfx + "time_feature1.", tidx, d_te)
    red.timefeat(p, g, pfx + "time_feature1_.", tidx, d_teb)
    red.timefeat(p, g, pfx + "time_feature2.", tidx, d_tes, spg=True)
    red.keep.append((sv, hp1, hp2, hp3, hp4, cp1, cp2, dout))
    return dd


class EncIn:

    def __init__(self, source, mask, fill, Wbt, ab, wv):
        self.source, self.mask, self.fill, self.Wbt, self.ab, self.wv = source, mask, fill, Wbt, ab, wv


ENCIN = os.environ.get("GPTST_ENCIN", "1") == "1"


def encin_ok(dims, base):
    return ENCIN and base == 1 and dims[3] in (64, 128) and dims[1] == 12 and chain_ok(dims)


GUIDEIN = os.environ.get("GPTST_GUIDEIN", "1") == "1"
GUIDE_HEAD = os.environ.get("GPTST_GUIDE_HEAD", "1") == "1"


class LowRankIn(NamedTuple):
    Wspa: Any


class GuideSaved(NamedTuple):
    t4m: Any
    spa: Any
    tem: Any
    h2: Any
    label: Any


def guide_fwd(p, source, tidx, dims, base, gen=None, lowrank_in=False):
    B, T, N, C = dims
    if gen is None:
        gen = gen_all(p, tidx, dims, which=(), guide=True).guide
    t4m, Wspa, bspa, Wtem, btem = gen
    m = "encoder.MLP_RL."
    if lowrank_in and GUIDEIN and GUIDE_HEAD and base == 1 and C == 64:
        r = ops.guide_head_fwd(source, p[m + "ln1.weight"], p[m + "ln1.bias"], Wspa, bspa, Wtem, btem, p[m + "ln3.weight"], p[m + "ln3.bias"])
        if r is not None:
            h1, h2, prob, label = r
            return prob, GuideSaved(t4m, LowRankIn(Wspa), CondLinSaved(h1, h2, Wtem), h2, label)
    if lowrank_in and GUIDEIN and base == 1 and C in (64, 128):
        h1 = ops.guide_in_fwd(source, p[m + "ln1.weight"], p[m + "ln1.bias"], Wspa, bspa)
        s1 = LowRankIn(Wspa)
    else:
        h0 = ops.lin_in(source, base + 2, base, p[m + "ln1.weight"], p[m + "ln1.bias"], C)
        h1, s1 = condlin_fwd(h0, Wspa, bspa, MODE_NODE, dims)
    h2, s2 = condlin_fwd(h1, Wtem, btem, MODE_TIME, dims)
    prob, label = ops.rowdot(h2, p[m + "ln3.weight"], p[m + "ln3.bias"], softmax=True, want_label=True)
    return prob, GuideSaved(t4m, s1, s2, h2, label)


def _wb_view(gw, gb):
    n = gw.numel() + gb.numel()
    if gb.data_ptr() != gw.data_ptr() + 4 * gw.numel():
        return None
    return torch.as_strided(gw, (1, n), (n, 1))


def fused_tails_ok(p, C, base, HS):
    return (C in (64, 128) and base <= ops.TAIL_MAXJ and HS <= ops.TAIL_MAXJ
            and _wb_view(p["decoder.dim_flow_out.weight"], p["decoder.dim_flow_out.bias"]) is not None
            and _wb_view(p["encoder.MLP_RL.ln3.weight"], p["encoder.MLP_RL.ln3.bias"]) is not None)


def loss_tail(p, g, dec, source, mask, base, sigma, mu, thresh, sws, red, chain=False):
    wo = "decoder.dim_flow_out."
    out, dd, part = ops.tail_mae(dec, p[wo + "weight"], p[wo + "bias"], source, base + 2, mask, sigma, mu, thresh, sws, premul=chain)
    red.jobs.bwd_pool(_ones(dec.device, part.shape[0]), part, _wb_view(g[wo + "weight"], g[wo + "bias"]))
    red.keep.append((part, dd))
    return out, dd


def kl_head(p, g, sv_g, prob, c1, N, w, sws, red, chain=False, carried=None):
    m = "encoder.MLP_RL."
    dh2, part = carried if carried is not None else ops.tail_kl(sv_g.h2, p[m + "ln3.weight"], prob, c1, N, w, sws, premul=chain)
    red.jobs.bwd_pool(_ones(prob.device, part.shape[0]), part, _wb_view(g[m + "ln3.weight"], g[m + "ln3.bias"]))
    red.keep.append((part, dh2))
    return dh2


def _linear_out_bwd(p, g, pfx, h, dy, C, chain, d_h=None):
    J = dy.shape[1]
    dh = ops.lin_in(dy, J, J, p[pfx + "weight"], None, C, wlayout=1)
    ops.rowouter(dy, J, J, h, g[pfx + "weight"], 1, asum=g[pfx + "bias"])
    if d_h is not None:
        dh = dh + d_h
    if chain:
        dh = dh * torch.where(h > 0, 1.0, 0.01)
    return dh


def guide_bwd(p, g, source, tidx, saved, dlogit, dims, base, red, dh2=None, chain=False, carried=None):
    B, T, N, C = dims
    carried = carried or KlOut()
    t4m, s1, s2, h2 = saved.t4m, saved.spa, saved.tem, saved.h2
    m = "encoder.MLP_RL."
    if dh2 is None:
        dh2 = _linear_out_bwd(p, g, m + "ln3.", h2, dlogit, C, chain)
    d_t4m = _zeros(t4m, *t4m.shape)
    dh1 = condlin_bwd(s2, dh2, t4m, p[m + "weights_pool_tem"], p[m + "bias_pool_tem"], g[m + "weights_pool_tem"],
                      g[m + "bias_pool_tem"], d_t4m, MODE_TIME, dims, red, chain, True, carried=carried.tem)
    if isinstance(s1, LowRankIn):
        assert chain
        neb, wpool, bpool = p["encoder.neb4mask"], p[m + "weights_pool_spa"], p[m + "bias_pool_spa"]
        K = neb.shape[1]
        dWb, dinp = carried.inp if carried.inp is not None else ops.guide_in_bwd(dh1, source, p[m + "ln1.weight"], p[m + "ln1.bias"], s1.Wspa)
        w = _wb_parts(dWb, C)
        red.jobs.bwd_pool(neb, w.dW, g[m + "weights_pool_spa"].view(K, C * C))
        red.jobs.bwd_pool(neb, w.db, g[m + "bias_pool_spa"])
        red.jobs.bwd_emb(w.dW, wpool.view(K, C * C), g["encoder.neb4mask"])
        red.jobs.bwd_emb(w.db, bpool, g["encoder.neb4mask"])
        wb = _wb_view(g[m + "ln1.weight"], g[m + "ln1.bias"])
        if wb is not None:
            red.jobs.bwd_pool(_ones(dh1.device, N), dinp, wb)
        else:
            g[m + "ln1.weight"].add_(dinp[:, :C].sum(0).view(C, 1))
            g[m + "ln1.bias"].add_(dinp[:, C:].sum(0))
        red.keep.append((dWb, dinp))
        dh0 = None
    else:
        dh0 = condlin_bwd(s1, dh1, p["encoder.neb4mask"], p[m + "weights_pool_spa"], p[m + "bias_pool_spa"],
                          g[m + "weights_pool_spa"], g[m + "bias_pool_spa"], g["encoder.neb4mask"], MODE_NODE, dims, red, chain, False)
        _in_proj_grads(source, base, dh0, g[m + "ln1.weight"], g[m + "ln1.bias"], None, 0.0, red)
    red.timefeat(p, g, GUIDE_TF, tidx, d_t4m)
    red.keep.append((saved, dlogit, dh2, dh1, dh0))


def kl_carry_ok(dims, HS, sv_g):
    B, T, N, C = dims
    return (CARRY_KL and C == 64 and T == 12 and HS <= ops.TAIL_MAXJ and chain_fwd_ok(dims) and chain_ok(dims)
            and sv_g is not None and isinstance(sv_g.spa, LowRankIn))


class KlOut:

    def __init__(self):
        self.head = None
        self.tem = None
        self.inp = None


class KlCarry:

    def __init__(self, p, sv_g, prob, source, dims, w, sws):
        self.p, self.sv_g, self.prob, self.source, self.dims, self.w, self.sws = p, sv_g, prob, source, dims, w, sws
        self.c1 = None
        self.stage = 0
        self.out = KlOut()

    def guest(self):
        if self.c1 is None or self.stage == 3:
            return None
        B, T, N, C = self.dims
        m = "encoder.MLP_RL."
        p, sv_g, dev = self.p, self.sv_g, self.prob.device
        HS = self.prob.shape[1]
        st = self.stage + 1
        f = dict(device=dev, dtype=torch.float32)
        if st == 1:
            h2, W3 = sv_g.h2, p[m + "ln3.weight"]
            dh2 = torch.empty_like(h2)
            part = torch.empty(ops.tail_parts(B * T * N), HS * C + HS, **f)
            self.out.head = (dh2, part)
            ts = [h2, W3, self.prob, self.c1, dh2, part, self.sws]
        elif st == 2:
            h1, Wtem = sv_g.tem.x, sv_g.tem.W
            dh2, _ = self.out.head
            ns = _C.lib().value("gptst_apply_wgrad_nsplit", MODE_TIME, B * T, N)
            dh1, dW, db = torch.empty_like(h1), torch.empty(ns * B * T, C * C, **f), torch.empty(ns * B * T, C, **f)
            self.out.tem = (dh1, WgradParts(dW, ns, db))
            ts = [dh2, h1, Wtem, dh1, dW, db]
        else:
            dh1, _ = self.out.tem
            dWb, dinp = torch.empty(N, C * C + C, **f), torch.empty(N, 2 * C, **f)
            self.out.inp = (dWb, dinp)
            ts = [dh1, self.source, p[m + "ln1.weight"], p[m + "ln1.bias"], sv_g.spa.Wspa, dWb, dinp]
        self.stage = st
        return (st, ts, 0, ops.kl_guest_blocks(st, B, T, N), HS, self.source.shape[-1], self.w)


def _in_proj_grads(source, base, dY, gW, gb, mask, fill, red):
    wb = _wb_view(gW, gb)
    if base == 1 and wb is not None:
        C = dY.shape[1]
        part = ops.rowouter_part(source, base + 2, base, dY, mask=mask, fill=fill)
        red.jobs.bwd_pool(_ones(dY.device, part.shape[0]), part[:, :2 * C], wb)
        red.keep.append(part)
    else:
        ops.rowouter(source, base + 2, base, dY, gW, 0, csum=gb, mask=mask, fill=fill)


class Forward(NamedTuple):
    emb: Any
    c1: Any
    dec: Any
    out: Any
    sv_e: Any
    sv_d: Any


def autoencoder_fwd(p, source, mask, dims, base, num_route, scaler_zeros, gen=None, tidx=None, lowrank_in=False, kl=None, head=True,
                    decoder=True, join=True):
    B, T, N, C = dims
    if tidx is None:
        tidx = source[:, :, 0, base:base + 2].contiguous()
    gen_e, gen_d = (gen.sthcn[ENC], gen.sthcn[DEC] if decoder else None) if gen is not None else (None, None)
    first = None
    if lowrank_in and gen_e is not None and encin_ok(dims, base):
        w, bi = p["encoder.dim_in_flow.weight"], p["encoder.dim_in_flow.bias"]
        G1, Wbt1, bbt1 = gen_e.ht(0)
        o1, ab, wv = ops.encin_ht1_fwd(source, base, mask, 0.0 if mask is None else scaler_zeros, w, bi, G1, Wbt1, bbt1)
        first = (o1.view(-1, C), EncIn(source, mask, 0.0 if mask is None else scaler_zeros, Wbt1, ab, wv))
        x0 = None
    else:
        x0 = ops.lin_in(source, base + 2, base, p["encoder.dim_in_flow.weight"], p["encoder.dim_in_flow.bias"], C,
                        mask=mask, fill=scaler_zeros)
    emb, c1, sv_e, dec_h1 = sthcn_fwd(p, ENC, tidx, x0, dims, num_route, gen=gen_e, head=first, next_gen=gen_d if join else None, kl=kl)
    if not decoder:
        return Forward(emb, c1, None, None, sv_e, None)
    dec, _, sv_d, _ = sthcn_fwd(p, DEC, tidx, emb, dims, num_route, gen=gen_d, head=dec_h1, kl=kl)
    out = ops.rowdot(dec, p["decoder.dim_flow_out.weight"], p["decoder.dim_flow_out.bias"]) if head else None
    return Forward(emb, c1, dec, out, sv_e, sv_d)


def model_bwd(p, g, source, mask, tidx, sv_e, sv_d, dec, d_out, d_dec, dims, base, scaler_zeros, red, dd=None, chain=False):
    B, T, N, C = dims
    if dd is None:
        dd = _linear_out_bwd(p, g, "decoder.dim_flow_out.", dec, d_out, C, chain, d_h=d_dec)
    defer = (chain and (red.on_bucket is None or PAIR_UNDER_DP) and not isinstance(sv_d.h1, EncIn)
             and ht_pair_ok(sv_d.h1, sv_e.h4, dims))
    late = defer and red.on_bucket is not None
    d_emb = sthcn_bwd(p, g, DEC, tidx, sv_d, dd, dims, red, chain, True, defer_h1=defer)
    if not late:
        red.flush_async(tidx)
    d_x0 = sthcn_bwd(p, g, ENC, tidx, sv_e, d_emb, dims, red, chain, False,
                     after_pending=(lambda: red.flush_async(tidx)) if late else None)
    red.flush_async(tidx)
    if d_x0 is not None:
        _in_proj_grads(source, base, d_x0, g["encoder.dim_in_flow.weight"], g["encoder.dim_in_flow.bias"], mask, scaler_zeros, red)


def step_bwd(p, g, source, mask, tidx, fw, prob, sv_g, dims, base, scaler_zeros, red, loss, stats, sws=None, with_kl=False, kl=None):
    B, T, N, C = dims
    sigma, mu, thresh = loss
    if sws is not None:
        chain = chain_ok(dims)
        done = kl.out if kl is not None else KlOut()
        _, dd = loss_tail(p, g, fw.dec, source, mask, base, sigma, mu, thresh, sws, red, chain=chain)
        model_bwd(p, g, source, mask, tidx, fw.sv_e, fw.sv_d, fw.dec, None, None, dims, base, scaler_zeros, red, dd=dd, chain=chain)
        if with_kl:
            dh2 = kl_head(p, g, sv_g, prob, fw.c1, N, 0.1, sws, red, chain=chain, carried=done.head)
            guide_bwd(p, g, source, tidx, sv_g, None, dims, base, red, dh2=dh2, chain=chain, carried=done)
    else:
        M = B * T * N
        ops.mae_fwd(fw.out, source, base + 2, mask, sigma, mu, thresh, M, base, stats)
        d_out = ops.mae_bwd(fw.out, source, base + 2, mask, sigma, mu, thresh, M, base, stats, normalize=False)
        model_bwd(p, g, source, mask, tidx, fw.sv_e, fw.sv_d, fw.dec, d_out, None, dims, base, scaler_zeros, red)
        if with_kl:
            dlogit = ops.kl(prob, fw.c1, N, 0.1, stats)
            guide_bwd(p, g, source, tidx, sv_g, dlogit, dims, base, red)


def module_bwd(p, g, source, mask, tidx, fw, prob, sv_g, dims, base, scaler_zeros, red, d_out, d_dec=None, d_prob=None, chain=False):
    model_bwd(p, g, source, mask, tidx, fw.sv_e, fw.sv_d, fw.dec, d_out, d_dec, dims, base, scaler_zeros, red, chain=chain)
    if d_prob is not None:
        dlogit = (prob * (d_prob - (d_prob * prob).sum(-1, keepdim=True))).contiguous()
        guide_bwd(p, g, source, tidx, sv_g, dlogit, dims, base, red, chain=chain)


def warm_up(fn):
    s = torch.cuda.Stream()
    s.wait_stream(torch.cuda.current_stream())
    with torch.cuda.stream(s):
        for _ in range(2):
            fn()
    torch.cuda.current_stream().wait_stream(s)
    torch.cuda.synchronize()
```

### gpt-st_amd/ops.py

```python
import ctypes
from typing import Any, NamedTuple

import torch

from . import _C

MODE_TIME, MODE_NODE, MODE_SHARED = 0, 1, 2
PRO_NONE, PRO_DPRE = 0, 1
EPI_PLAIN, EPI_RES_LRELU, EPI_ADD_DPRE, EPI_LRELU, EPI_ADD_PREMUL, EPI_PREMUL = 0, 1, 2, 3, 4, 5

_p = _C.ptr


TIMER = None
LAST_CALL = {}


CALL_LOCK = None


def _call(name, *args, tag="", nbytes=0):
    if CALL_LOCK is not None:
        with CALL_LOCK:
            _C.lib().call(name, *args, _C.stream())
# ... 114 lines not shown
        self.jobs.append(PoolJob(self.FWD, emb, None, pool, out, R, K, pool.numel() // K, 1, 0))
        return out

    def gram(self, emb, pool, out, A=None):
        _chk(emb, pool, out, A)
        R, K = emb.shape
        cols = pool.numel() // K
        assert cols % 12 == 0 and out.numel() == R * 144 and out.is_contiguous()
        if _C.lib().value("gptst_pool_jobs_gram_rows", K, cols) <= 0:
            assert A is not None and A.numel() == R * cols, "gram job does not fit and no forward output was given"
            self.post.append((A, out, R, cols // 12))
            return out
        self.jobs.append(PoolJob(self.GRAM, emb, None, pool, out, R, K, cols, 1, 0))
        return out

    @staticmethod
    def _ldx(dW, cols):
        assert dW.is_cuda and dW.dtype == torch.float32 and dW.dim() == 2 and dW.shape[1] == cols and dW.stride(1) == 1, (dW.shape, dW.stride(), cols)
        return dW.stride(0)

    def bwd_pool(self, emb, dW, dpool, nsplit=1):
        _chk(emb, dpool)
        R, K = emb.shape
        cols = dpool.numel() // K
        self.jobs.append(PoolJob(self.BWD_POOL, emb, dW, None, dpool, R, K, cols, nsplit, self._ldx(dW, cols)))

    def bwd_emb(self, dW, pool, demb, nsplit=1):
        _chk(pool, demb)
        R, K = demb.shape
        cols = pool.numel() // K
        self.jobs.append(PoolJob(self.BWD_EMB, None, dW, pool, demb, R, K, cols, nsplit, self._ldx(dW, cols)))

    @staticmethod
    def columns(js, fields=PoolJob._fields):
        return [len(js)] + [(_ptrs0 if f in ("emb", "dW", "pool", "out") else _ints)([getattr(j, f) for j in js])
                            for f in PoolJob._fields if f in fields]

    def launch(self):
        js, self.jobs = self.jobs, []
        post, self.post = self.post, []
        if js:
            _call("gptst_pool_jobs", *self.columns(js), nbytes=_nb(*[t for j in js for t in (j.emb, j.dW, j.pool, j.out)]))
        for A, G, rows, Hm in post:
            _call("gptst_gram_fwd", _p(A), _p(G), rows, Hm)


def _ptrs0(ts):
    return (ctypes.c_void_p * len(ts))(*[(t.data_ptr() if t is not None else None) for t in ts])


def apply(A, W, mode, BT, N, bias=None, resid=None, A2=None, transw=False, pro=PRO_NONE, epi=EPI_PLAIN, colsum=None,
          out=None, resid2=None):
    _chk(A, W, bias, resid, A2, resid2)
    C = A.shape[-1]
    if out is None:
        out = torch.empty_like(A)
    cs, ns = None, 0
    if colsum is not None:
        G = BT if mode == MODE_TIME else (N if mode == MODE_NODE else 1)
        ns = _C.lib().value("gptst_apply_nsplit", mode, BT, N, C)
        cs = torch.empty(ns * G, C, device=A.device, dtype=torch.float32)
    _call("gptst_apply", _p(A), _p(A2), _p(W), int(W.dim() == 3), int(transw), _p(bias), _p(resid), _p(resid2), _p(out), _p(cs),
          mode, pro, epi, BT, N, C, tag="mode%d pro%d epi%d" % (mode, pro, epi), nbytes=_nb(A, A2, W, bias, resid, resid2, out))
    if colsum is True:
        return out, cs, ns
    if colsum is not None:
        colsum.add_(cs.view(ns, -1, C).sum(0).view_as(colsum))
    return out


def apply_wgrad(dOut, Y, S, W, mode, BT, N, premul=False):
    _chk(dOut, Y, S, W)
    C = dOut.shape[-1]
    G = BT if mode == MODE_TIME else N
    ns = _C.lib().value("gptst_apply_wgrad_nsplit", mode, BT, N)
    dS = torch.empty_like(dOut)
    dW = torch.empty(ns * G, C * C, device=dOut.device, dtype=torch.float32)
    db = torch.empty(ns * G, C, device=dOut.device, dtype=torch.float32)
    _call("gptst_apply_wgrad", _p(dOut), _p(Y), _p(S), _p(W), _p(dS), _p(dW), _p(db), int(premul), mode, BT, N, C, tag="mode%d" % mode,
          nbytes=_nb(dOut, Y, S, W, dS, dW))
    return dS, dW, db, ns


def linear_bwd(dY, X, Wp, dOut, out, premul=False):
    _chk(dY, X, Wp, dOut, out)
    rows, C = dY.shape
    ns = _C.lib().value("gptst_linear_bwd_nsplit", rows)
    dX = torch.empty_like(dY)
    dWp = torch.empty(ns, C * C, device=dY.device, dtype=torch.float32)
    dbp = torch.empty(ns, C, device=dY.device, dtype=torch.float32)
    _call("gptst_linear_bwd", _p(dY), _p(X), _p(Wp), _p(dOut), _p(out), _p(dX), _p(dWp), _p(dbp), int(premul), rows, C,
          nbytes=_nb(dY, X, dOut, out, dX, dWp))
    return dX, dWp, dbp, ns


def wgrad_nsplit(mode, BT, N, C=64):
    return _C.lib().value("gptst_wgrad_nsplit", mode, BT, N, C)


def wgrad(A, D, mode, BT, N, D2=None, pro=PRO_NONE, colsum_a=False, colsum_d=False):
    _chk(A, D, D2)
    C = A.shape[-1]
    ns = wgrad_nsplit(mode, BT, N, C)
    G = BT if mode == MODE_TIME else (N if mode == MODE_NODE else 1)
    if colsum_a or colsum_d:
        dW = torch.empty(ns * G, C * C + C, device=A.device, dtype=torch.float32)
        _call("gptst_wgrad_colsum", _p(A), _p(D), _p(D2), _p(dW), mode, pro, 1 if colsum_a else 2, BT, N, C,
              tag="mode%d pro%d cs" % (mode, pro), nbytes=_nb(A, D, D2, dW))
    else:
        dW = torch.empty(ns * G, C, C, device=A.device, dtype=torch.float32)
        _call("gptst_wgrad", _p(A), _p(D), _p(D2), _p(dW), mode, pro, BT, N, C, tag="mode%d pro%d" % (mode, pro), nbytes=_nb(A, D, D2, dW))
    return dW, ns


def gram_fwd(A):
    N, Hm, T = A.shape
    G = torch.empty(N, T, T, device=A.device, dtype=torch.float32)
    _call("gptst_gram_fwd", _p(A), _p(G), N, Hm)
    return G


def gram_bwd(A, dG, out=None, layers=1, nsplit=1):
    LN, Hm, T = A.shape
    dA = out if out is not None else torch.empty_like(A)
    _call("gptst_gram_bwd", _p(A), _p(dG), _p(dA), layers, LN // layers, Hm, nsplit)
    return dA


def tmix(X, G, dOut=None, Y=None):
    _chk(X, G, dOut, Y)
    B, T, N, C = X.shape
    out = torch.empty_like(X)
    _call("gptst_tmix", _p(X), _p(G), _p(dOut), _p(Y), _p(out), B, T, N, C, tag="bwd" if dOut is not None else "fwd",
          nbytes=_nb(X, G, dOut, Y, out))
    return out


def hypertem_fwd(X, G, Wbt, bbt, want_R=True):
    _chk(X, G, Wbt, bbt)
    B, T, N, C = X.shape
    R = torch.empty_like(X) if want_R else None
    out = torch.empty_like(X)
    _call("gptst_hypertem_fwd", _p(X), _p(G), _p(Wbt), _p(bbt), _p(R), _p(out), B, T, N, C, nbytes=_nb(X, G, Wbt, bbt, R, out))
    return R, out


def hypertem_chain_fwd(X, stages, want_R=True, guest=None):
    B, T, N, C = X.shape
    _chk(X, *[t for st in stages for t in st])
    f = lambda: torch.empty(B, T, N, C, device=X.device, dtype=torch.float32)
    Rs = [f() if want_R else None for _ in stages]
    outs = [f() for _ in stages]
    chain = (_p(X), len(stages), _ptrs0([st[0] for st in stages]), _ptrs0([st[1] for st in stages]), _ptrs0([st[2] for st in stages]),
             _ptrs0(Rs), _ptrs0(outs), B, T, N, C)
    if guest is None:
        _call("gptst_hypertem_chain_fwd", *chain, tag="x%d" % len(stages), nbytes=_nb(X, *Rs, *outs))
    else:
        stage, ts, v0, v1, HS, lda, w = guest
        _chk(*ts)
        _call("gptst_hypertem_chain_fwd_kl", *chain, stage, _ptrs0(ts), v0, v1, HS, lda, float(w), tag="x%d+kl%d" % (len(stages), stage),
              nbytes=_nb(X, *Rs, *outs))
    return list(zip(Rs, outs))


def kl_guest_blocks(stage, B, T, N):
    return _C.lib().value("gptst_kl_guest_blocks", stage, B, T, N)


def encin_ht1_fwd(source, base, mask, fill, w, bi, G, Wbt, bbt):
    B, T, N, F = source.shape
    C = Wbt.shape[-1]
    assert base == 1
    _chk(source, mask, w, bi, G, Wbt, bbt)
    f = dict(device=source.device, dtype=torch.float32)
    out, ab, wv = torch.empty(B, T, N, C, **f), torch.empty(B * T * N, 2, **f), torch.empty(B * T, 2 * C, **f)
    _call("gptst_encin_ht1_fwd", _p(source), F, _p(mask), float(fill), _p(w), _p(bi), _p(G), _p(Wbt), _p(bbt), _p(out), _p(ab), _p(wv), B, T, N, C,
          nbytes=_nb(Wbt, out))
    return out, ab, wv


def encin_ht1_bwd(dPre, source, mask, fill, w, bi, Wbt, ab, wv, dG=None):
    B, T, N, F = source.shape
    C = Wbt.shape[-1]
    _chk(dPre, source, mask, w, bi, Wbt, ab, wv, dG)
    f = dict(device=source.device, dtype=torch.float32)
    dWb, dinp = torch.empty(B * T, C * C + C, **f), torch.empty(B * T, 2 * C, **f)
    if dG is None:
        dG = torch.empty(B, N, T, T, **f)
    _call("gptst_encin_ht1_bwd", _p(dPre), _p(source), F, _p(mask), float(fill), _p(w), _p(bi), _p(Wbt), _p(ab), _p(wv), _p(dWb), _p(dG), _p(dinp),
          B, T, N, C, nbytes=_nb(dPre, Wbt, dWb, dG))
    return dWb, dG, dinp


def guide_in_fwd(source, w1, b1, Wn, bn):
    B, T, N, F = source.shape
    C = Wn.shape[-1]
    _chk(source, w1, b1, Wn, bn)
    h1 = torch.empty(B * T * N, C, device=source.device, dtype=torch.float32)
    _call("gptst_guide_in_fwd", _p(source), F, _p(w1), _p(b1), _p(Wn), _p(bn), _p(h1), B * T, N, C, nbytes=_nb(Wn, h1))
    return h1


def guide_head_fwd(source, w1, b1, Wn, bn, Wbt, bbt, W3, b3):
    B, T, N, F = source.shape
    C, J = Wn.shape[-1], W3.shape[0]
    if C != 64 or J > 16:
        return None
    _chk(source, w1, b1, Wn, bn, Wbt, bbt, W3, b3)
    dev = source.device
    f = dict(device=dev, dtype=torch.float32)
    uc = torch.empty(N, 2 * C, **f)
    h1, h2 = torch.empty(B * T * N, C, **f), torch.empty(B * T * N, C, **f)
    prob = torch.empty(B * T * N, J, **f)
    label = torch.empty(B * T * N, device=dev, dtype=torch.int32)
    _call("gptst_guide_head_fwd", _p(source), F, _p(w1), _p(b1), _p(Wn), _p(bn), _p(Wbt), _p(bbt), _p(W3), _p(b3), _p(uc), _p(h1), _p(h2), _p(prob),
          _p(label), B * T, N, C, J, nbytes=_nb(Wbt, h1, h2, prob))
    return h1, h2, prob, label


def guide_in_bwd(dPre, source, w1, b1, Wn):
    B, T, N, F = source.shape
    C = Wn.shape[-1]
    _chk(dPre, source, w1, b1, Wn)
    f = dict(device=source.device, dtype=torch.float32)
    dWb, dinp = torch.empty(N, C * C + C, **f), torch.empty(N, 2 * C, **f)
    _call("gptst_guide_in_bwd", _p(dPre), _p(source), F, _p(w1), _p(b1), _p(Wn), _p(dWb), _p(dinp), B * T, N, C, nbytes=_nb(dPre, Wn, dWb))
    return dWb, dinp


def hypertem_ntiles(N):
    return _C.lib().value("gptst_hypertem_ntiles", N)


def hypertem_bwd(dOut, Y, X, G, Wbt, dG=None, want_dbias=True, premul=False):
    _chk(dOut, Y, X, G, Wbt, dG)
    B, T, N, C = X.shape
    dX = torch.empty_like(X)
    nt = hypertem_ntiles(N)
    dbias = torch.empty(nt * B * T, C, device=X.device, dtype=torch.float32) if want_dbias else None
    if dG is None:
        dG = torch.empty(B, N, T, T, device=X.device, dtype=torch.float32)
    _call("gptst_hypertem_bwd", _p(dOut), _p(Y), _p(X), _p(G), _p(Wbt), _p(dX), _p(dbias), _p(dG), int(premul), B, T, N, C,
          nbytes=_nb(dOut, Y, X, G, Wbt, dX))
    return dX, dbias, dG


def hypertem_bwd_wgrad(dOut, Y, X, G, Wbt, R, dG=None, premul=False):
    _chk(dOut, Y, X, G, Wbt, R, dG)
    B, T, N, C = X.shape
    dX = torch.empty_like(X)
    if dG is None:
        dG = torch.empty(B, N, T, T, device=X.device, dtype=torch.float32)
    ns = wgrad_nsplit(MODE_TIME, B * T, N, C)
    dWb = torch.empty(ns * B * T, C * C + C, device=X.device, dtype=torch.float32)
    _call("gptst_hypertem_bwd_wgrad", _p(dOut), _p(Y), _p(X), _p(G), _p(Wbt), _p(R), _p(dX), _p(dG), _p(dWb), int(premul), B, T, N, C,
          nbytes=_nb(dOut, Y, X, G, Wbt, R, dX, dWb))
    return dX, dWb, ns, dG


def hypertem_bwd_pair(dOut1, X1, G1, Wbt1, R1, X0, G0, Wbt0, R0, dG1, dG0, cnt, dWb1=None):
    _chk(dOut1, X1, G1, Wbt1, R1, X0, G0, Wbt0, R0, dG1, dG0, cnt, dWb1)
    B, T, N, C = X1.shape
    if C != 64:
        return None
    dXmid, dX0 = torch.empty_like(X1), torch.empty_like(X0)
    ns = wgrad_nsplit(MODE_TIME, B * T, N, C)
    dWb0 = torch.empty(ns * B * T, C * C + C, device=X1.device, dtype=torch.float32)
    if dWb1 is None:
        dWb1 = torch.empty_like(dWb0)
    assert dWb1.shape == dWb0.shape
    try:
        _call("gptst_hypertem_bwd_pair", _p(dOut1), _p(X1), _p(G1), _p(Wbt1), _p(R1), _p(X0), _p(G0), _p(Wbt0), _p(R0), _p(dXmid), _p(dX0),
              _p(dG1), _p(dG0), _p(dWb1), _p(dWb0), _p(cnt), B, T, N, C, nbytes=_nb(dOut1, X1, R1, X0, R0, dXmid, dX0, dWb0, dWb1))
    except _C.GptstError as e:
        if e.code != _C.ESHAPE:
            raise
        return None
    return dXmid, dX0, dWb1, dWb0, ns


def tmix_bwd(dR, X, G, dOut, Y, dG=None):
    _chk(dR, X, G, dOut, Y, dG)
    B, T, N, C = X.shape
    dX = torch.empty_like(X)
    if dG is None:
        dG = torch.empty(N, T, T, device=X.device, dtype=torch.float32)
    _call("gptst_tmix_bwd", _p(dR), _p(X), _p(G), _p(dOut), _p(Y), _p(dX), _p(dG), B, T, N, C, nbytes=_nb(dR, X, dOut, Y, dX))
    return dX, dG


def tmix_bwd_chain(dR, X, G, dPre, premul=False, dG=None):
    _chk(dR, X, G, dPre, dG)
    B, T, N, C = X.shape
    dX = torch.empty_like(X)
    if dG is None:
        dG = torch.empty(N, T, T, device=X.device, dtype=torch.float32)
    _call("gptst_tmix_bwd_chain", _p(dR), _p(X), _p(G), _p(dPre), int(bool(premul)), _p(dX), _p(dG), B, T, N, C, nbytes=_nb(dR, X, dPre, dX))
    return dX, dG


# ... 510 lines not shown
```

### gpt-st_amd/step.py

```python
import contextlib
import math
import os
import random
from typing import Any, NamedTuple

import torch

from . import engine, ops

DEFER_GEN = os.environ.get("GPTST_DEFER_GEN", "1") == "1"
U24 = os.environ.get("GPTST_MASK_U24", "1") == "1"


class Part1(NamedTuple):
    tidx: Any
    gen: Any
    red: Any
    prob: Any
    sv_g: Any


class PretrainStep:
    RING = 8
    DETERMINISTIC_MODE = True
# ... 112 lines not shown
            red.on_bucket = self._bucket_ready
            red.bucket_inline, red.fork_side = True, self.fork_side
        lowrank = self.fused_tails and engine.chain_ok(dims)
        prob, sv_g = engine.guide_fwd(p, src, tidx, dims, base, gen=gen.guide, lowrank_in=lowrank) if need_guide else (None, None)
        if self._needs_exchange(phase):
            self.label_l.copy_(sv_g.label)
        return Part1(tidx, gen, red, prob, sv_g)

    def _part2(self, phase, ctx):
        if not self.safe_mode:
            return self._part2_impl(phase, ctx)
        with engine.no_handoffs():
            return self._part2_impl(phase, ctx)

    def _part2_impl(self, phase, ctx):
        mdl, p, g, dims, base = self.model, self.model.param_views(), self.g, self.dims, self.base
        a = self.args
        src, tidx, gen, red, prob, sv_g = self.src, ctx.tidx, ctx.gen, ctx.red, ctx.prob, ctx.sv_g
        engine.CTX.ARENA, engine.CTX.NODE_REDUCE = self.arena, self.node_reduce
        pend = gen.pending
        mask = self._make_mask(phase, prob, sv_g.label if sv_g is not None else None, pend)
        if pend is not None:
            pend.launch()
        self.last_mask = mask
        fused = self.fused_tails
        kl, sws = None, None
        if phase == 1 and self._carry_kl(sv_g):
            sws = self._tail_sws()
            kl = engine.KlCarry(p, sv_g, prob, src, dims, 0.1, sws)
        fw = engine.autoencoder_fwd(p, src, mask, dims, base, mdl.num_route, mdl.scaler_zeros, gen=gen, tidx=tidx,
                                    lowrank_in=fused and engine.chain_ok(dims), kl=kl, head=not fused, join=self.join_enc_dec)
        if fused and sws is None:
            sws = self._tail_sws()
        engine.step_bwd(p, g, src, mask, tidx, fw, prob, sv_g, dims, base, mdl.scaler_zeros, red, (self.std, self.mean, a.mape_thresh),
                        self.stats, sws=sws, with_kl=phase == 1, kl=kl)
        self._fold_stats(sws)
        red.flush(tidx)
        engine.CTX.ARENA = engine.CTX.NODE_REDUCE = None
        self._after_backward(phase)

    def _noise_buffer(self, phase):
        if self.gmask:
            return self.noise_g if phase == 0 else self.noise_ar_g
        return self.noise if phase == 0 else self.noise_ar

    def _need_guide(self, phase):
        return phase == 1 or self.always_guide

    def _make_mask(self, phase, prob, label, pend):
        a, base, M = self.args, self.base, self.B * self.T * self.N
        if self.gmask:
            return self._global_mask(phase, jobs=pend)
        if self.force_mask:
            return self.mask_buf
        if phase == 0:
            return ops.mask_random(self.noise, int(M * base * a.mask_ratio), ws=self._mask_ws(), u24=U24, jobs=pend)
        return ops.mask_adaptive(label, None, self.ctrl[:self.HS], self.ctrl[self.HS:], self.noise_a, self.noise_r,
                                 a.ada_type == "all", base, ws=self._mask_ws(), u24=U24, jobs=pend)[2]

    def _fold_stats(self, sws):
        if sws is None:
            return
        if self.dp is None:
            self._sws = sws
        else:
            ops.stats_fold(sws, self.stats)

    def _after_backward(self, phase):
        if self.dp is None:
            self._optim()
        elif self._dp_in_graph():
            if self._dec_reduced:
                self._allreduce(self.gbuf[:self.dec_lo])
                self._allreduce(self.gbuf[self.dec_hi:])
            else:
                self._allreduce(self.gbuf)
            self._optim()

    def _tail_sws(self):
        return self.arena.zeros(ops.tail_parts(self.B * self.T * self.N), 4)

    def _carry_kl(self, sv_g):
        return (self.fused_tails and self.dp is None and not self.global_count_scale and not self.deterministic and not self.safe_mode
                and not self.always_guide and engine.CTX.NODE_REDUCE is None and engine.kl_carry_ok(self.dims, self.HS, sv_g))

    def _mask_ws(self):
        return self.arena.zeros(ops.mask_ws_floats())

    def _global_mask(self, phase, jobs=None):
        a, base, M = self.args, self.base, self.B * self.T * self.N
        Mg = M * self.W
        if self.force_mask:
            return self.mask_buf
        if phase == 0:
            mask_g = ops.mask_random(self.noise_g, int(Mg * base * a.mask_ratio), ws=self._mask_ws(), u24=U24, jobs=jobs)
        else:
            mask_g = ops.mask_adaptive(self.label_g, None, self.ctrl[:self.HS], self.ctrl[self.HS:], self.noise_a_g,
                                       self.noise_r_g, a.ada_type == "all", base, ws=self._mask_ws(), u24=U24, jobs=jobs)[2]
        self.last_mask_global = mask_g
        return self.dp.rows_of(mask_g, M * base)

    def _exchange_labels(self):
        self.dp.gather_labels(self.label_l, out=self.label_g)

    def _optim(self):
        sws, self._sws = self._sws, None
        ops.clip_adam(self.model.flat, self.gflat, self.m, self.v, self.model.nA, self.model.nB, self.hyper, self.stats,
                      stats_out=self.stats_out, sws=sws)

    @contextlib.contextmanager
    def _launch_mode(self):
        if self.DETERMINISTIC_MODE:
            ops.set_deterministic(self.deterministic)
        try:
            yield
        finally:
            if self.DETERMINISTIC_MODE:
                ops.set_deterministic(False)
            engine.CTX.ARENA = engine.CTX.NODE_REDUCE = None

    def _enqueue(self, phase):
        ctx = self._part1(phase)
        if self._needs_exchange(phase):
            self._exchange_labels()
        self._part2(phase, ctx)

    def _body(self, phase):
        with self._launch_mode():
            self._enqueue(phase)

    def _views(self, hc):
        HS = self.HS
        n = hc.numpy()
        return dict(hc=hc, hyper=n[:16].view("float32"), ctrl=n[16:16 + HS + 2], rng=n[16 + HS + 2:], ev=None)

    def _slot(self):
        sl = self._ring[self._ring_i]
        self._ring_i = (self._ring_i + 1) % self.RING
        if sl["ev"] is not None:
            sl["ev"].synchronize()
        return sl

    def _host_prepare(self, phase, epoch, list_c):
        sl = self._slot()
        self._fill(sl, phase, epoch, list_c)
        self.hc.copy_(sl["hc"], non_blocking=True)
        if sl["ev"] is None:
            sl["ev"] = torch.cuda.Event()
        sl["ev"].record()

    def _fill(self, sl, phase, epoch, list_c):
        a = self.args
        self.tA += 1
        if phase == 1:
            self.tB += 1
        self.phase_kl = phase == 1
        b1, b2 = 0.9, 0.999
        tA, tB = self.tA, self.tB
        sl["hyper"][11:13] = (1 - b1, 1 - b2)
        sl["hyper"][:11] = (self.lr / (1 - b1 ** tA), math.sqrt(1 - b2 ** tA),
                            self.lr / (1 - b1 ** tB) if tB else 0.0, math.sqrt(1 - b2 ** tB) if tB else 1.0,
                            b1, b2, 1e-8, float(a.max_grad_norm) if a.grad_norm else 0.0, 1.0 if phase == 1 else 0.0,
                            1.0,
                            1.0)
        sl["rng"][:2] = (self.noise_seed & 0x7FFFFFFF, tA & 0x7FFFFFFF)
        if phase == 1:
            if list_c is None:
# ... 289 lines not shown
```

### include/gptst_hip.h

```cpp
#ifndef GPTST_HIP_H
#define GPTST_HIP_H
#include <stdint.h>

#ifdef __cplusplus
extern "C" {
#endif
#if defined(__GNUC__)
#pragma GCC visibility push(default)
#endif

#define GPTST_ABI_VERSION 16
int gptst_abi_version(void);
int gptst_set_deterministic(int on);
int gptst_handoff_timeouts(int* out);
int gptst_handoff_reset(void);
int gptst_mask_cooperative(int on);
int gptst_mask_cooperative_state(void);
int gptst_set_handoff_guard(int on);

int gptst_poolgen_fwd(const float* emb, const float* pool, float* out, int cols, const float* pool2, float* out2,
                      int cols2, int R, int K, void* stream);
int gptst_poolgen_bwd_pool(const float* emb, const float* dW, float* dpool, int cols, const float* dW2, float* dpool2,
                           int cols2, int R, int nsplit, int K, void* stream);
int gptst_poolgen_bwd_emb(const float* dW, const float* pool, int cols, const float* dW2, const float* pool2, int cols2,
                          float* demb, int R, int nsplit, int K, void* stream);

int gptst_poolgen_fwd_multi(const float* emb, int nprob, const void* pools, const void* outs, const int* cols, int R, int K,
                            void* stream);
int gptst_poolgen_bwd_pool_multi(const float* emb, int nprob, const void* dWs, const void* dpools, const int* cols, const int* nsplit,
                                 int R, int K, void* stream);
int gptst_poolgen_bwd_emb_multi(int nprob, const void* dWs, const void* pools, const int* cols, const int* nsplit, float* demb, int R,
                                int K, void* stream);

int gptst_pool_jobs(int njobs, const int* kind, const void* const* emb, const void* const* x, const void* const* pool,
                    const void* const* out, const int* R, const int* K, const int* cols, const int* nsplit, const int* ldx, void* stream);
int gptst_pool_jobs_gram_rows(int K, int cols);

int gptst_apply_nsplit(int mode, int BT, int N, int C);
int gptst_apply(const float* A, const float* A2, const float* W, int w_per_group, int transw, const float* bias,
                const float* resid, const float* resid2, float* out, float* colsum, int mode, int pro, int epi, int BT,
                int N, int C, void* stream);
int gptst_wgrad_nsplit(int mode, int BT, int N, int C);
int gptst_wgrad(const float* A, const float* D, const float* D2, float* dW, int mode, int pro, int BT, int N, int C,
                void* stream);
int gptst_wgrad_colsum(const float* A, const float* D, const float* D2, float* dW, int mode, int pro, int which, int BT, int N, int C,
                       void* stream);

int gptst_apply_wgrad_nsplit(int mode, int BT, int N);
int gptst_apply_wgrad(const float* dOut, const float* Y, const float* S, const float* W, float* dS, float* dW, float* colsum, int premul,
                      int mode, int BT, int N, int C, void* stream);

int gptst_linear_bwd_nsplit(int rows);
int gptst_linear_bwd(const float* dY, const float* X, const float* Wp, const float* dOut, const float* out, float* dX, float* dWp, float* dbp,
                     int premul, int rows, int C, void* stream);

int gptst_gram_fwd(const float* A, float* G, int N, int Hm, void* stream);
int gptst_gram_bwd(const float* A, const float* dG, float* dA, int L, int N, int Hm, int nsplit, void* stream);
int gptst_tmix(const float* X, const float* G, const float* dOut, const float* Y, float* out, int B, int T, int N, int C,
               void* stream);
int gptst_tmix_dgraph(const float* dR, const float* X, float* dG, int B, int T, int N, int C, void* stream);
int gptst_tmix_bwd(const float* dR, const float* X, const float* G, const float* dOut, const float* Y, float* dX, float* dG, int B, int T,
                   int N, int C, void* stream);
int gptst_tmix_bwd_chain(const float* dR, const float* X, const float* G, const float* dPre, int premul, float* dX, float* dG, int B, int T,
                         int N, int C, void* stream);

int gptst_hypertem_fwd(const float* X, const float* G, const float* Wbt, const float* bbt, float* R_out, float* out, int B, int T,
                       int N, int C, void* stream);
int gptst_hypertem_chain_fwd(const float* X, int nstage, const void* Gs, const void* Wbts, const void* bbts, const void* Rs, const void* outs,
                             int B, int T, int N, int C, void* stream);
int gptst_hypertem_chain_fwd_kl(const float* X, int nstage, const void* Gs, const void* Wbts, const void* bbts, const void* Rs, const void* outs,
                                int B, int T, int N, int C, int stage, const void* ops, int v0, int v1, int HS, int lda, float w, void* stream);
int gptst_kl_guest_blocks(int stage, int B, int T, int N);

int gptst_encin_ht1_fwd(const float* src, int lda, const float* mask, float fill, const float* w, const float* bi, const float* G,
                        const float* Wbt, const float* bbt, float* out, float* ab, float* wv, int B, int T, int N, int C, void* stream);
int gptst_encin_ht1_bwd(const float* dPre, const float* src, int lda, const float* mask, float fill, const float* w, const float* bi,
                        const float* Wbt, const float* ab, const float* wv, float* dWb, float* dG, float* dinp, int B, int T, int N, int C,
                        void* stream);

int gptst_guide_in_fwd(const float* src, int lda, const float* w1, const float* b1, const float* Wn, const float* bn, float* h1, int BT, int N,
                       int C, void* stream);
int gptst_guide_in_bwd(const float* dPre, const float* src, int lda, const float* w1, const float* b1, const float* Wn, float* dWb, float* dinp,
                       int BT, int N, int C, void* stream);
int gptst_guide_uc_floats(int N, int C);
int gptst_guide_head_fwd(const float* src, int lda, const float* w1, const float* b1, const float* Wn, const float* bn, const float* Wbt,
                         const float* bbt, const float* W3, const float* b3, float* uc, float* h1, float* h2, float* prob, int* label,
                         int BT, int N, int C, int J, void* stream);

int gptst_hypertem_ntiles(int N);
int gptst_hypertem_bwd(const float* dOut, const float* Y, const float* X, const float* G, const float* Wbt, float* dX, float* dbias,
                       float* dG, int premul, int B, int T, int N, int C, void* stream);
int gptst_hypertem_bwd_wgrad(const float* dOut, const float* Y, const float* X, const float* G, const float* Wbt, const float* R, float* dX,
                             float* dG, float* dWb, int premul, int B, int T, int N, int C, void* stream);
int gptst_hypertem_bwd_pair(const float* dOut1, const float* X1, const float* G1, const float* Wbt1, const float* R1, const float* X0,
                            const float* G0, const float* Wbt0, const float* R0, float* dXmid, float* dX0, float* dG1, float* dG0,
                            float* dWb1, float* dWb0, void* cnt, int B, int T, int N, int C, void* stream);

int gptst_cap_route_fwd(const float* X, const float* Wp, const float* bp, const float* dadj, float* c_out, float* s_out, int BT, int N,
                        int C, int HS, int R, void* stream);
int gptst_cap_cross_fwd(const float* s, const float* dyn, const float* tmpl, float* v, float* Ht, float* Rt, int B, int T, int C,
                        int HS, int HT, void* stream);
int gptst_cap_cross_ws_floats(int B, int T, int C, int HS, int HT);
int gptst_cap_cross_bwd(const float* dv, const float* s, const float* Rt, const float* Ht, const float* dyn, const float* tmpl,
                        float* dS, float* ddyn, float* ws, int B, int T, int C, int HS, int HT, void* stream);
int gptst_cap_rec_fwd(const float* c, const float* v, float* rec, int BT, int N, int C, int HS, void* stream);
int gptst_cap_cross_rec_fwd(const float* s, const float* dyn, const float* tmpl, const float* c, float* v, float* Ht, float* Rt, float* rec,
                            int B, int T, int N, int C, int HS, int HT, void* stream);
int gptst_cap_rec_bwd(const float* drec, const float* c, const float* v, float* dc1, float* dv, int BT, int N, int C, int HS,
                      void* stream);
int gptst_cap_route_bwd(const float* X, const float* Wp, const float* bp, const float* c, const float* dc1, const float* dS,
                        float* dY, float* dlogit, int BT, int N, int C, int HS, void* stream);
int gptst_cap_cross_route_bwd(const float* X, const float* Wp, const float* bp, const float* c, const float* dc1, const float* dv,
                              const float* s, const float* Rt, const float* Ht, const float* dyn, const float* tmpl, float* dY,
                              float* dlogit, float* ddyn, float* dS_ws, void* flags, int B, int T, int N, int C, int HS, int HT, void* stream);
int gptst_cap_cross_route_lin_bwd(const float* X, const float* Wp, const float* bp, const float* c, const float* dc1, const float* dv,
                                  const float* s, const float* Rt, const float* Ht, const float* dyn, const float* tmpl,
                                  const float* dPre, const float* out, int premul, float* dX, float* dWp, float* dbp, float* dlogit,
                                  float* ddyn, float* dS_ws, void* flags, int B, int T, int N, int C, int HS, int HT, void* stream);
int gptst_cap_route_roles_ok(int B, int T, int N, int C, int HS, int HT);
int gptst_cap_cross_route_lin_bwd_jobs(const float* X, const float* Wp, const float* bp, const float* c, const float* dc1, const float* dv,
                                       const float* s, const float* Rt, const float* Ht, const float* dyn, const float* tmpl,
                                       const float* dPre, const float* out, int premul, float* dX, float* dWp, float* dbp, float* dlogit,
                                       float* ddyn, float* dS_ws, void* flags, int B, int T, int N, int C, int HS, int HT,
                                       int njobs, const int* jkind, const void* const* jemb, const void* const* jx, const void* const* jpool,
                                       const void* const* jout, const int* jR, const int* jK, const int* jcols, const int* jnsplit, const int* jldx,
                                       void* stream);
int gptst_cap_split_units(int BT, int N, int C, int HS);
int gptst_cap_cross_route_lin_bwd_split(const float* X, const float* Wp, const float* bp, const float* c, const float* dc1, const float* dv,
                                        const float* s, const float* Rt, const float* Ht, const float* dyn, const float* tmpl,
                                        const float* dPre, const float* out, int premul, float* dX, float* dWp, float* dbp, float* dlogit,
                                        float* ddyn, float* dS_ws, void* flags, int B, int T, int N, int C, int HS, int HT, int nsplit,
                                        int njobs, const int* jkind, const void* const* jemb, const void* const* jx, const void* const* jpool,
                                        const void* const* jout, const int* jR, const int* jK, const int* jcols, const int* jnsplit, const int* jldx,
                                        void* stream);

int gptst_cap_fits_lds(int N, int C, int HS);
int gptst_capbig_squash_rows(float* Y, long rows, int C, void* stream);
int gptst_capbig_softmax(const float* bl, const float* l0, float* cs, int BT, int HS, int N, int use_bl, int use_l0, void* stream);
int gptst_capbig_type1(const float* cs, const float* P, float* S, int BT, int HS, int N, int C, void* stream);
int gptst_capbig_post(const float* S, const float* V0, float* out, long rows, int C, int post, void* stream);
int gptst_capbig_type2(const float* V, const float* P, float* bl, int BT, int HS, int N, int C, void* stream);
int gptst_capbig_rec_fwd(const float* c, const float* v, float* rec, int BT, int HS, int N, int C, void* stream);
int gptst_capbig_rec_bwd_dc(const float* drec, const float* v, float* dc1, int BT, int HS, int N, int C, void* stream);
int gptst_capbig_route_bwd_rows(const float* Y, const float* c, const float* dc1, const float* dS, float* dY, float* dlogit, int BT,
                                int HS, int N, int C, void* stream);

int gptst_capflow_supported(int HS, int C);
int gptst_capflow_nparts(int N);
int gptst_capflow_squash(const float* Y, const float* dadj, float* P, float* part, int BT, int HS, int N, int C, void* stream);
int gptst_capflow_route(const float* rows, const float* V, const float* bl_in, float* bl_out, const float* l0, const float* c_in,
                        float* c_out, float* part, int BT, int HS, int N, int C, void* stream);
int gptst_capflow_post(const float* part, int nparts, int prow, float* V0, float* Vout, int mode, int BT, int HS, int C, void* stream);
int gptst_capflow_rec_fwd(const float* c, const float* v, float* rec, int BT, int HS, int N, int C, void* stream);
int gptst_capflow_route_bwd(const float* Y, const float* c, const float* dc1, const float* dS, float* dY, float* dlogit, int BT,
// ... 111 lines not shown
```

Before: 927.6 steps/s.

## Recompute guide h1 from source and uc in backward, add hypertem KL guest host

The guide head forward can now skip storing its time-conditioned hidden activation h1. The backward apply-wgrad kernel rebuilds h1 on the fly from the source scalar and the per-node uc vectors (fma plus leaky-ReLU) instead of reading a full BT*N*C tensor. The KL guest plan now splits stage 2 into shares across chain hosts and adds the single hypertem forward kernel as a host for stage 3 guest blocks. This trades an activation write and read for a little recompute and more overlap of the KL path, at the cost of extra scheduling complexity and LDS traffic inside the rebuilt kernel.

```diff
diff --git a/gpt-st_amd/csrc/apply.hip b/gpt-st_amd/csrc/apply.hip
--- a/gpt-st_amd/csrc/apply.hip
+++ b/gpt-st_amd/csrc/apply.hip
@@ -289,14 +289,14 @@
     wgrad64_body<PRO, U>(A, D, D2, dW, rm, rows_per_split, ostride, csa, blockIdx.x, blockIdx.y, smem);
 }
 
-template <int KIND, int CHAIN>
+template <int KIND, int CHAIN, bool REB = false>
 __global__ __launch_bounds__(256, 2) void applywg64_kernel(const float* __restrict__ dOut, const float* __restrict__ Y,
                                                             const float* __restrict__ S, const float* __restrict__ W, long w_gstride,
                                                             const float* __restrict__ resid, const float* __restrict__ resid2,
                                                             float* __restrict__ dS, float* __restrict__ dW, float* __restrict__ colsum,
-                                                            RowMap rm, int tiles_per_wave) {
+                                                            RowMap rm, int tiles_per_wave, LowRankS lr) {
     __shared__ __attribute__((aligned(16))) float lds[APPLYWG64_LDS_FLOATS];
-    applywg64_body<KIND, CHAIN>(dOut, Y, S, W, w_gstride, resid, resid2, dS, dW, colsum, rm, tiles_per_wave, blockIdx.x, blockIdx.y, lds);
+    applywg64_body<KIND, CHAIN, REB>(dOut, Y, S, W, w_gstride, resid, resid2, dS, dW, colsum, rm, tiles_per_wave, blockIdx.x, blockIdx.y, lds, lr);
 }
 
 GPTST_INTERNAL int gptst_apply_wgrad_geometry(int mode, int BT, int N, int* tpw) {
@@ -322,9 +322,23 @@
     apply64_geometry(rm, false, tpw, gy);
     const dim3 grid(rm.G, gy);
     hipStream_t st = (hipStream_t)stream;
-    if (Y) hipLaunchKernelGGL((applywg64_kernel<0, 0>), grid, dim3(256), 0, st, dOut, Y, S, W, (long)C * C, nullptr, nullptr, dS, dW, colsum, rm, tpw);
-    else if (!premul) hipLaunchKernelGGL((applywg64_kernel<0, 1>), grid, dim3(256), 0, st, dOut, Y, S, W, (long)C * C, nullptr, nullptr, dS, dW, colsum, rm, tpw);
-    else hipLaunchKernelGGL((applywg64_kernel<0, 2>), grid, dim3(256), 0, st, dOut, Y, S, W, (long)C * C, nullptr, nullptr, dS, dW, colsum, rm, tpw);
+    const LowRankS none{};
+    if (Y) hipLaunchKernelGGL((applywg64_kernel<0, 0>), grid, dim3(256), 0, st, dOut, Y, S, W, (long)C * C, nullptr, nullptr, dS, dW, colsum, rm, tpw, none);
+    else if (!premul) hipLaunchKernelGGL((applywg64_kernel<0, 1>), grid, dim3(256), 0, st, dOut, Y, S, W, (long)C * C, nullptr, nullptr, dS, dW, colsum, rm, tpw, none);
+    else hipLaunchKernelGGL((applywg64_kernel<0, 2>), grid, dim3(256), 0, st, dOut, Y, S, W, (long)C * C, nullptr, nullptr, dS, dW, colsum, rm, tpw, none);
+    GPTST_CHECK_LAUNCH();
+    return GPTST_OK;
+}
+
+extern "C" int gptst_apply_wgrad_guide(const float* dOut, const float* src, int lda, const float* uc, const float* W, float* dS, float* dW,
+                                       float* colsum, int BT, int N, int C, void* stream) {
+    if (!dOut || !src || !uc || !W || !dS || !dW || BT <= 0 || N <= 0 || lda <= 0) return GPTST_EARG;
+    if (C != 64) return GPTST_ESHAPE;
+    RowMap rm = make_rowmap(0, BT, N);
+    int tpw, gy;
+    apply64_geometry(rm, false, tpw, gy);
+    hipLaunchKernelGGL((applywg64_kernel<0, 2, true>), dim3(rm.G, gy), dim3(256), 0, (hipStream_t)stream, dOut, nullptr, nullptr, W, (long)C * C, nullptr,
+                       nullptr, dS, dW, colsum, rm, tpw, LowRankS{src, lda, uc});
     GPTST_CHECK_LAUNCH();
     return GPTST_OK;
 }
@@ -344,9 +358,10 @@
     int tpw, gy;
     apply64_geometry(rm, false, tpw, gy);
     hipStream_t st = (hipStream_t)stream;
-    if (out) hipLaunchKernelGGL((applywg64_kernel<1, 0>), dim3(1, gy), dim3(256), 0, st, dY, nullptr, X, Wp, 0L, dOut, out, dX, dWp, dbp, rm, tpw);
-    else if (!premul) hipLaunchKernelGGL((applywg64_kernel<1, 1>), dim3(1, gy), dim3(256), 0, st, dY, nullptr, X, Wp, 0L, dOut, nullptr, dX, dWp, dbp, rm, tpw);
-    else hipLaunchKernelGGL((applywg64_kernel<1, 2>), dim3(1, gy), dim3(256), 0, st, dY, nullptr, X, Wp, 0L, dOut, X, dX, dWp, dbp, rm, tpw);
+    const LowRankS none{};
+    if (out) hipLaunchKernelGGL((applywg64_kernel<1, 0>), dim3(1, gy), dim3(256), 0, st, dY, nullptr, X, Wp, 0L, dOut, out, dX, dWp, dbp, rm, tpw, none);
+    else if (!premul) hipLaunchKernelGGL((applywg64_kernel<1, 1>), dim3(1, gy), dim3(256), 0, st, dY, nullptr, X, Wp, 0L, dOut, nullptr, dX, dWp, dbp, rm, tpw, none);
+    else hipLaunchKernelGGL((applywg64_kernel<1, 2>), dim3(1, gy), dim3(256), 0, st, dY, nullptr, X, Wp, 0L, dOut, X, dX, dWp, dbp, rm, tpw, none);
     GPTST_CHECK_LAUNCH();
     return GPTST_OK;
 }
diff --git a/gpt-st_amd/csrc/guidein.hip b/gpt-st_amd/csrc/guidein.hip
--- a/gpt-st_amd/csrc/guidein.hip
+++ b/gpt-st_amd/csrc/guidein.hip
@@ -108,6 +108,7 @@
 
 #define GH_P 68
 extern thread_local int g_apply_tpw;
+template <bool ST1>
 __global__ __launch_bounds__(256, 2) void guide_head_fwd_kernel(const float* __restrict__ src, int lda, const float* __restrict__ uc,
                                                                 const float* __restrict__ Wbt, const float* __restrict__ bbt,
                                                                 const float* __restrict__ W3, const float* __restrict__ b3,
@@ -150,7 +151,8 @@
         for (int q = 0; q < 4; ++q) {
             float4 y = f4fma(sn, un[q], cn[q]);
             y.x = lrelu(y.x); y.y = lrelu(y.y); y.z = lrelu(y.z); y.w = lrelu(y.w);
-            if (mrow < N) st4(h1 + ((size_t)g * N + mrow) * C + 16 * q + 4 * kk, y); else y = f4zero();
+            if (mrow >= N) y = f4zero();
+            else if (ST1) st4(h1 + ((size_t)g * N + mrow) * C + 16 * q + 4 * kk, y);
             a[q] = y;
         }
         if (t + 1 < t1) fetch(t + 1);
@@ -209,7 +211,7 @@
 extern "C" int gptst_guide_head_fwd(const float* src, int lda, const float* w1, const float* b1, const float* Wn, const float* bn, const float* Wbt,
                                     const float* bbt, const float* W3, const float* b3, float* uc, float* h1, float* h2, float* prob, int* label,
                                     int BT, int N, int C, int J, void* stream) {
-    if (!src || !w1 || !b1 || !Wn || !bn || !Wbt || !bbt || !W3 || !b3 || !uc || !h1 || !h2 || !prob || !label || BT <= 0 || N <= 0 || lda <= 0 || J <= 0)
+    if (!src || !w1 || !b1 || !Wn || !bn || !Wbt || !bbt || !W3 || !b3 || !uc || !h2 || !prob || !label || BT <= 0 || N <= 0 || lda <= 0 || J <= 0)
         return GPTST_EARG;
     if (C != 64 || J > 16) return GPTST_ESHAPE;
     hipLaunchKernelGGL((guide_uc_kernel<64>), dim3(N), dim3(256), 0, (hipStream_t)stream, w1, b1, Wn, bn, uc);
@@ -218,7 +220,8 @@
     if (g_apply_tpw > 0) tpw = g_apply_tpw;
     if (tpw < 1) tpw = 1;
     const int gy = (ntiles + 4 * tpw - 1) / (4 * tpw);
-    hipLaunchKernelGGL(guide_head_fwd_kernel, dim3(BT, gy), dim3(256), 0, (hipStream_t)stream, src, lda, uc, Wbt, bbt, W3, b3, h1, h2, prob, label, N, J, tpw);
+    if (h1) hipLaunchKernelGGL(guide_head_fwd_kernel<true>, dim3(BT, gy), dim3(256), 0, (hipStream_t)stream, src, lda, uc, Wbt, bbt, W3, b3, h1, h2, prob, label, N, J, tpw);
+    else hipLaunchKernelGGL(guide_head_fwd_kernel<false>, dim3(BT, gy), dim3(256), 0, (hipStream_t)stream, src, lda, uc, Wbt, bbt, W3, b3, h1, h2, prob, label, N, J, tpw);
     GPTST_CHECK_LAUNCH();
     return GPTST_OK;
 }
diff --git a/gpt-st_amd/csrc/hypertem.hip b/gpt-st_amd/csrc/hypertem.hip
--- a/gpt-st_amd/csrc/hypertem.hip
+++ b/gpt-st_amd/csrc/hypertem.hip
@@ -34,10 +34,11 @@
     return 16;
 }
 
+template <int GUEST>
 __global__ __launch_bounds__(256, HT_OCC) void hypertem_fwd_kernel(const float* __restrict__ X, const float* __restrict__ G,
                                                               const float* __restrict__ Wbt, const float* __restrict__ bbt,
                                                               float* __restrict__ R_out, float* __restrict__ out, int N, int B, int NT,
-                                                              int dbg) {
+                                                              int dbg, KlGuest kg) {
     constexpr int C = 64, P = C + 4, GP = 145;
     int tsi = 0;
 #ifdef GPTST_DEBUG
@@ -49,6 +50,9 @@
     extern __shared__ __attribute__((aligned(16))) float smem[];
     float* Xs = smem;
     float* Gs = Xs + HT_T * NT * P;
+    if constexpr (GUEST != 0) {
+        if ((int)blockIdx.x >= kg.base) { kl_guest_run<GUEST>(kg, kg.v0 + (int)blockIdx.x - kg.base, smem); return; }
+    }
     int b, tile;
     if (!ht_work((N + NT - 1) / NT, B, b, tile)) return;
     const int n0 = tile * NT;
@@ -138,15 +142,45 @@
 }
 
 static size_t ht_smem(int NT) { return ((size_t)HT_T * NT * 68 + NT * 145) * sizeof(float); }
+static int ht_fwd_grid(int B, int N, int NT) { return 8 * ((B + 7) / 8) * ((N + NT - 1) / NT); }
 
 extern "C" int gptst_hypertem_fwd(const float* X, const float* G, const float* Wbt, const float* bbt, float* R_out, float* out, int B,
                                   int T, int N, int C, void* stream) {
     if (!X || !G || !Wbt || !bbt || !out || T != HT_T) return GPTST_EARG;
     if (C != 64) return GPTST_ESHAPE;
     static int done = 0;
-    if (!done) { hipFuncSetAttribute((const void*)hypertem_fwd_kernel, hipFuncAttributeMaxDynamicSharedMemorySize, (int)ht_smem(16)); done = 1; }
+    if (!done) { hipFuncSetAttribute((const void*)hypertem_fwd_kernel<0>, hipFuncAttributeMaxDynamicSharedMemorySize, (int)ht_smem(16)); done = 1; }
     const int NT = ht_pick_nt(B, N);
-    hipLaunchKernelGGL(hypertem_fwd_kernel, dim3(8 * ((B + 7) / 8) * ((N + NT - 1) / NT)), dim3(256), ht_smem(NT), (hipStream_t)stream, X, G, Wbt, bbt, R_out, out, N, B, NT, g_ht_dbg);
+    const KlGuest none{};
+    hipLaunchKernelGGL(hypertem_fwd_kernel<0>, dim3(ht_fwd_grid(B, N, NT)), dim3(256), ht_smem(NT), (hipStream_t)stream, X, G, Wbt, bbt, R_out, out, N, B, NT, g_ht_dbg, none);
+    GPTST_CHECK_LAUNCH();
+    return GPTST_OK;
+}
+
+extern "C" int gptst_kl_guest_blocks(int stage, int B, int T, int N);
+extern "C" int gptst_hypertem_fwd_kl(const float* X, const float* G, const float* Wbt, const float* bbt, float* R_out, float* out, int B, int T,
+                                     int N, int C, int stage, const void* ops, int v0, int v1, int HS, int lda, float w, void* stream) {
+    if (!X || !G || !Wbt || !bbt || !out || T != HT_T || !ops || stage < 1 || stage > 3) return GPTST_EARG;
+    if (C != 64 || stage != 3) return GPTST_ESHAPE;
+    (void)HS; (void)w;
+    if (v0 < 0 || v1 <= v0 || v1 > gptst_kl_guest_blocks(stage, B, T, N) || lda <= 0) return GPTST_EARG;
+    const float* const* p = (const float* const*)ops;
+    for (int i = 0; i < 7; ++i) if (!p[i]) return GPTST_EARG;
+    const int NT = ht_pick_nt(B, N);
+    KlGuest kg{};
+    kg.base = ht_fwd_grid(B, N, NT);
+    kg.v0 = v0;
+    kg.dPre = p[0]; kg.src = p[1]; kg.lda = lda; kg.w1 = p[2]; kg.b1 = p[3]; kg.Wn = p[4]; kg.dWb = (float*)p[5]; kg.dinp = (float*)p[6];
+    kg.BT = B * T; kg.N = N;
+    const size_t sg = kl_guest_lds_bytes(stage), sh = ht_smem(NT);
+    const int smem = (int)(sg > sh ? sg : sh);
+    static int done = 0;
+    if (!done) {
+        const size_t s16 = ht_smem(16);
+        (void)hipFuncSetAttribute((const void*)hypertem_fwd_kernel<3>, hipFuncAttributeMaxDynamicSharedMemorySize, (int)(sg > s16 ? sg : s16));
+        done = 1;
+    }
+    hipLaunchKernelGGL(hypertem_fwd_kernel<3>, dim3(kg.base + (v1 - v0)), dim3(256), smem, (hipStream_t)stream, X, G, Wbt, bbt, R_out, out, N, B, NT, g_ht_dbg, kg);
     GPTST_CHECK_LAUNCH();
     return GPTST_OK;
 }
@@ -796,7 +830,7 @@
     const int nv = gptst_kl_guest_blocks(stage, B, T, N);
     if (v0 < 0 || v1 <= v0 || v1 > nv) return GPTST_EARG;
     const float* const* p = (const float* const*)ops;
-    const int np = stage == 1 ? 7 : stage == 2 ? 6 : 7;
+    const int np = 7;
     for (int i = 0; i < np; ++i) if (!p[i]) return GPTST_EARG;
     KlGuest kg{};
     kg.base = ht_chain_grid(B, N);
@@ -807,9 +841,10 @@
         t.rows = B * T * N; t.J = HS; t.N = N; t.w = w; t.premul = 1;
         gptst_tail_geometry(t.rows, &t.rows_per_block);
     } else if (stage == 2) {
-        kg.dOut = p[0]; kg.S = p[1]; kg.W = p[2]; kg.dS = (float*)p[3]; kg.dW = (float*)p[4]; kg.colsum = (float*)p[5];
+        if (lda <= 0) return GPTST_EARG;
+        kg.dOut = p[0]; kg.src = p[1]; kg.lda = lda; kg.uc = p[2]; kg.W = p[3]; kg.dS = (float*)p[4]; kg.dW = (float*)p[5]; kg.colsum = (float*)p[6];
         kg.rm = make_rowmap(0, B * T, N);
-        gptst_apply_wgrad_geometry(0, B * T, N, &kg.tpw);
+        kg.ns = gptst_apply_wgrad_geometry(0, B * T, N, &kg.tpw);
     } else {
         if (lda <= 0) return GPTST_EARG;
         kg.dPre = p[0]; kg.src = p[1]; kg.lda = lda; kg.w1 = p[2]; kg.b1 = p[3]; kg.Wn = p[4]; kg.dWb = (float*)p[5]; kg.dinp = (float*)p[6];
diff --git a/gpt-st_amd/csrc/kl_guest.h b/gpt-st_amd/csrc/kl_guest.h
--- a/gpt-st_amd/csrc/kl_guest.h
+++ b/gpt-st_amd/csrc/kl_guest.h
@@ -166,11 +166,15 @@
 
 constexpr int APPLYWG64_LDS_FLOATS = 4 * 64 * 64 + 4 * 64;
 
-template <int KIND, int CHAIN>
+struct LowRankS { const float* src; int lda; const float* uc; };
+
+template <int KIND, int CHAIN, bool REB = false>
 __device__ __forceinline__ void applywg64_body(const float* __restrict__ dOut, const float* __restrict__ Y, const float* __restrict__ S,
                                                const float* __restrict__ W, long w_gstride, const float* __restrict__ resid,
                                                const float* __restrict__ resid2, float* __restrict__ dS, float* __restrict__ dW,
-                                               float* __restrict__ colsum, RowMap rm, int tiles_per_wave, int g, int split, float* __restrict__ lds) {
+                                               float* __restrict__ colsum, RowMap rm, int tiles_per_wave, int g, int split, float* __restrict__ lds,
+                                               LowRankS lr = LowRankS{}) {
+    static_assert(!REB || (KIND == 0 && CHAIN == 2), "the rebuilt operand serves the guide's time-conditioned layer only");
     constexpr int C = 64, TP = C + 4;
     float* smem = lds;
     float (*csl)[C] = reinterpret_cast<float (*)[C]>(lds + 4 * C * C);
@@ -181,16 +185,33 @@
     const int ntiles = (rm.M + 15) / 16;
     const int t0 = (split * 4 + wave) * tiles_per_wave, t1 = min(ntiles, t0 + tiles_per_wave);
     float4 d[4], y[4], a[4];
+    float sf[4];
+    float4 un[4], cn[4];
+    auto rebuild = [](float s, const float4& u, const float4& c) {
+        float4 v = f4fma(s, u, c);
+        v.x = lrelu(v.x); v.y = lrelu(v.y); v.z = lrelu(v.z); v.w = lrelu(v.w);
+        return v;
+    };
     auto fetch = [&](int t) {
 #pragma unroll
         for (int s4 = 0; s4 < 4; ++s4) {
             const int m = min(t * 16 + 4 * s4 + kk, rm.M - 1);
-            const size_t off = ((size_t)g * rm.rs_g + (size_t)m * rm.rs_m) * C + 4 * j;
-            d[s4] = ld4(dOut + off); a[s4] = ld4(S + off);
+            const size_t row = (size_t)g * rm.rs_g + (size_t)m * rm.rs_m;
+            const size_t off = row * C + 4 * j;
+            d[s4] = ld4(dOut + off);
+            if (REB) sf[s4] = lr.src[row * lr.lda];
+            else a[s4] = ld4(S + off);
             if (KIND == 0 && CHAIN == 0) y[s4] = ld4(Y + off);
         }
     };
-    if (t0 < t1) fetch(t0);
+    auto fetch_uc = [&](int t) {
+#pragma unroll
+        for (int s4 = 0; s4 < 4; ++s4) {
+            const int m = min(t * 16 + 4 * s4 + kk, rm.M - 1);
+            un[s4] = ld4(lr.uc + (size_t)m * 2 * C + 4 * j); cn[s4] = ld4(lr.uc + (size_t)m * 2 * C + C + 4 * j);
+        }
+    };
+    if (t0 < t1) { fetch(t0); if (REB) fetch_uc(t0); }
     load_w_lds<C, 256>(Wl, W + (size_t)g * w_gstride, KIND == 0 ? 1 : 0, threadIdx.x);
     __syncthreads();
     float4 bv[4][4];
@@ -207,6 +228,10 @@
     for (int t = t0; t < t1; ++t) {
         if (KIND == 1 && t != t0) fetch(t);
         SB();
+        if (REB) {
+#pragma unroll
+            for (int s4 = 0; s4 < 4; ++s4) a[s4] = rebuild(sf[s4], un[s4], cn[s4]);
+        }
 #pragma unroll
         for (int s4 = 0; s4 < 4; ++s4) {
             float4 v = d[s4];
@@ -231,9 +256,16 @@
 #pragma unroll
         for (int q = 0; q < 4; ++q) ap[q] = ld4(tile + j * TP + 16 * q + 4 * kk);
         const int tcur = t;
+        float4 rv[4], rv2[4];
+        if (REB) {
+#pragma unroll
+            for (int s4 = 0; s4 < 4; ++s4) st4(tile + (4 * s4 + kk) * TP + 4 * j, a[s4]);
+        }
         if (KIND == 0 && t + 1 < t1) fetch(t + 1);
-        float4 rv[4], rv2[4];
-        if (KIND == 1 || CHAIN == 2) {
+        if (REB) {
+#pragma unroll
+            for (int r = 0; r < 4; ++r) rv2[r] = ld4(tile + (4 * kk + r) * TP + 4 * j);
+        } else if (KIND == 1 || CHAIN == 2) {
 #pragma unroll
             for (int r = 0; r < 4; ++r) {
                 const int m = min(tcur * 16 + kk * 4 + r, rm.M - 1);
@@ -274,6 +306,7 @@
             }
             if (m < rm.M) st4(dS + ((size_t)g * rm.rs_g + (size_t)m * rm.rs_m) * C + 4 * j, o4);
         }
+        if (REB && t + 1 < t1) fetch_uc(t + 1);
     }
     cs.x += __shfl_xor(cs.x, 16, 64); cs.y += __shfl_xor(cs.y, 16, 64); cs.z += __shfl_xor(cs.z, 16, 64); cs.w += __shfl_xor(cs.w, 16, 64);
     cs.x += __shfl_xor(cs.x, 32, 64); cs.y += __shfl_xor(cs.y, 32, 64); cs.z += __shfl_xor(cs.z, 32, 64); cs.w += __shfl_xor(cs.w, 32, 64);
@@ -359,15 +392,15 @@
     int base;
     int v0;
     TailArgs tail;
-    const float* dOut; const float* S; const float* W; float* dS; float* dW; float* colsum; RowMap rm; int tpw;
+    const float* dOut; const float* uc; const float* W; float* dS; float* dW; float* colsum; RowMap rm; int tpw, ns;
     const float* dPre; const float* src; int lda; const float* w1; const float* b1; const float* Wn; float* dWb; float* dinp; int BT, N;
 };
 
 template <int STAGE>
 __device__ __forceinline__ void kl_guest_run(const KlGuest& k, int v, float* lds) {
     if constexpr (STAGE == 1) tail_mfma_body<1, 64>(k.tail, v, lds);
-    else if constexpr (STAGE == 2) applywg64_body<0, 2>(k.dOut, nullptr, k.S, k.W, 64L * 64, nullptr, nullptr, k.dS, k.dW, k.colsum, k.rm, k.tpw,
-                                                        v % k.rm.G, v / k.rm.G, lds);
+    else if constexpr (STAGE == 2) applywg64_body<0, 2, true>(k.dOut, nullptr, nullptr, k.W, 64L * 64, nullptr, nullptr, k.dS, k.dW, k.colsum, k.rm, k.tpw,
+                                                              v / k.ns, v % k.ns, lds, LowRankS{k.src, k.lda, k.uc});
     else guide_in_bwd_body<64>(k.dPre, k.src, k.lda, k.w1, k.b1, k.Wn, k.dWb, k.dinp, k.BT, k.N, v, lds);
 }
 
diff --git a/gpt-st_amd/engine.py b/gpt-st_amd/engine.py
--- a/gpt-st_amd/engine.py
+++ b/gpt-st_amd/engine.py
@@ -169,11 +169,12 @@
     return dims[3] == 64 and FUSE_HT_BWD
 
 
-def hypertem_core_fwd(x, G, Wbt, bbt, dims):
+def hypertem_core_fwd(x, G, Wbt, bbt, dims, kl=None):
     B, T, N, C = dims
     if C == 64:
         keep = not (DROP_R and _ht_fused_bwd(dims) and ops.wgrad_nsplit(MODE_TIME, B * T, N, C) == 1)
-        R, out = ops.hypertem_fwd(x.view(B, T, N, C), G, Wbt, bbt, want_R=keep)
+        R, out = ops.hypertem_fwd(x.view(B, T, N, C), G, Wbt, bbt, want_R=keep,
+                                  guest=kl.guest(KL_HOST_LAYER) if kl is not None else None)
         R, out = (R.view(-1, C) if keep else None), out.view(-1, C)
     else:
         R = ops.tmix(x.view(B, T, N, C), G).view(-1, C)
@@ -208,6 +209,10 @@
 def _genlin_bwd(dout, out, x, W, mode, dims, chain, premul=False):
     B, T, N, C = dims
     BT = B * T
+    if isinstance(x, ops.LowRankH1):
+        assert C == 64 and mode == MODE_TIME and chain and premul
+        dx, dW, db, ns = ops.apply_wgrad_guide(dout, x, W, BT, N)
+        return dx, WgradParts(dW, ns, db)
     if C == 64:
         dx, dW, db, ns = ops.apply_wgrad(dout, None if chain else out, x, W, mode, BT, N, premul=chain and premul)
         return dx, WgradParts(dW, ns, db)
@@ -358,7 +363,7 @@
 
 def ht_chain_fwd(x, stages, dims, kl=None):
     B, T, N, C = dims
-    res = ops.hypertem_chain_fwd(x.view(B, T, N, C), stages, guest=kl.guest() if kl is not None else None)
+    res = ops.hypertem_chain_fwd(x.view(B, T, N, C), stages, guest=kl.guest(KL_HOST_CHAIN) if kl is not None else None)
     saved, xin = [], x
     for (G, Wbt, _b), (R, o) in zip(stages, res):
         o = o.view(-1, C)
@@ -563,7 +568,7 @@
         (h4, h1n), xn = ht_chain_fwd(x, [ht(3), next_gen.ht(0)], dims, kl)
         x, nhead = h4.out, (xn, h1n)
     else:
-        x, h4 = hypertem_core_fwd(x, *ht(3), dims)
+        x, h4 = hypertem_core_fwd(x, *ht(3), dims, kl)
     return x, c1, SthcnSaved(h1, h2, h3, h4, sc1, sc2, gen.emb, gen, gen.slot), nhead
 
 
@@ -705,7 +710,8 @@
     t4m, Wspa, bspa, Wtem, btem = gen
     m = "encoder.MLP_RL."
     if lowrank_in and GUIDEIN and GUIDE_HEAD and base == 1 and C == 64:
-        r = ops.guide_head_fwd(source, p[m + "ln1.weight"], p[m + "ln1.bias"], Wspa, bspa, Wtem, btem, p[m + "ln3.weight"], p[m + "ln3.bias"])
+        r = ops.guide_head_fwd(source, p[m + "ln1.weight"], p[m + "ln1.bias"], Wspa, bspa, Wtem, btem, p[m + "ln3.weight"], p[m + "ln3.bias"],
+                               want_h1=False)
         if r is not None:
             h1, h2, prob, label = r
             return prob, GuideSaved(t4m, LowRankIn(Wspa), CondLinSaved(h1, h2, Wtem), h2, label)
@@ -796,10 +802,18 @@
     red.keep.append((saved, dlogit, dh2, dh1, dh0))
 
 
-def kl_carry_ok(dims, HS, sv_g):
-    B, T, N, C = dims
-    return (CARRY_KL and C == 64 and T == 12 and HS <= ops.TAIL_MAXJ and chain_fwd_ok(dims) and chain_ok(dims)
-            and sv_g is not None and isinstance(sv_g.spa, LowRankIn))
+KL_HOST_CHAIN, KL_HOST_LAYER = "chain", "layer"
+
+
+def kl_carry_ok(dims, HS, sv_g, join=True):
+    B, T, N, C = dims
+    return (CARRY_KL and C == 64 and T == 12 and HS <= ops.TAIL_MAXJ and chain_fwd_ok(dims) and chain_ok(dims) and join
+            and sv_g is not None and isinstance(sv_g.spa, LowRankIn) and isinstance(sv_g.tem.x, ops.LowRankH1))
+
+
+def kl_stage2_shares(groups, ns):
+    n, k = groups * ns, (groups + 1) // 2 * ns
+    return [(0, n)] if k >= n else [(0, k), (k, n)]
 
 
 class KlOut:
@@ -815,17 +829,24 @@
     def __init__(self, p, sv_g, prob, source, dims, w, sws):
         self.p, self.sv_g, self.prob, self.source, self.dims, self.w, self.sws = p, sv_g, prob, source, dims, w, sws
         self.c1 = None
-        self.stage = 0
+        B, T, N, C = dims
+        ns = _C.lib().value("gptst_apply_wgrad_nsplit", MODE_TIME, B * T, N)
+        self.plan = ([(KL_HOST_CHAIN, 1, 0, ops.kl_guest_blocks(1, B, T, N))] + [(KL_HOST_CHAIN, 2, a, b) for a, b in kl_stage2_shares(B * T, ns)]
+                     + [(KL_HOST_LAYER, 3, 0, ops.kl_guest_blocks(3, B, T, N))])
+        self.sent = 0
         self.out = KlOut()
 
-    def guest(self):
-        if self.c1 is None or self.stage == 3:
+    def done(self):
+        return self.sent == len(self.plan)
+
+    def guest(self, host):
+        if self.c1 is None or self.done() or self.plan[self.sent][0] != host:
             return None
         B, T, N, C = self.dims
         m = "encoder.MLP_RL."
         p, sv_g, dev = self.p, self.sv_g, self.prob.device
         HS = self.prob.shape[1]
-        st = self.stage + 1
+        _, st, v0, v1 = self.plan[self.sent]
         f = dict(device=dev, dtype=torch.float32)
         if st == 1:
             h2, W3 = sv_g.h2, p[m + "ln3.weight"]
@@ -834,19 +855,21 @@
             self.out.head = (dh2, part)
             ts = [h2, W3, self.prob, self.c1, dh2, part, self.sws]
         elif st == 2:
-            h1, Wtem = sv_g.tem.x, sv_g.tem.W
+            x, Wtem = sv_g.tem.x, sv_g.tem.W
             dh2, _ = self.out.head
-            ns = _C.lib().value("gptst_apply_wgrad_nsplit", MODE_TIME, B * T, N)
-            dh1, dW, db = torch.empty_like(h1), torch.empty(ns * B * T, C * C, **f), torch.empty(ns * B * T, C, **f)
-            self.out.tem = (dh1, WgradParts(dW, ns, db))
-            ts = [dh2, h1, Wtem, dh1, dW, db]
+            if v0 == 0:
+                ns = _C.lib().value("gptst_apply_wgrad_nsplit", MODE_TIME, B * T, N)
+                dh1, dW, db = torch.empty_like(dh2), torch.empty(ns * B * T, C * C, **f), torch.empty(ns * B * T, C, **f)
+                self.out.tem = (dh1, WgradParts(dW, ns, db))
+            dh1, w = self.out.tem
+            ts = [dh2, x.source, x.uc, Wtem, dh1, w.dW, w.db]
         else:
             dh1, _ = self.out.tem
             dWb, dinp = torch.empty(N, C * C + C, **f), torch.empty(N, 2 * C, **f)
             self.out.inp = (dWb, dinp)
             ts = [dh1, self.source, p[m + "ln1.weight"], p[m + "ln1.bias"], sv_g.spa.Wspa, dWb, dinp]
-        self.stage = st
-        return (st, ts, 0, ops.kl_guest_blocks(st, B, T, N), HS, self.source.shape[-1], self.w)
+        self.sent += 1
+        return (st, ts, v0, v1, HS, self.source.shape[-1], self.w)
 
 
 def _in_proj_grads(source, base, dY, gW, gb, mask, fill, red):
@@ -915,6 +938,7 @@
     sigma, mu, thresh = loss
     if sws is not None:
         chain = chain_ok(dims)
+        assert kl is None or kl.done(), "a KL-path stage found no host: kl_carry_ok promised all four (%d of %d sent)" % (kl.sent, len(kl.plan))
         done = kl.out if kl is not None else KlOut()
         _, dd = loss_tail(p, g, fw.dec, source, mask, base, sigma, mu, thresh, sws, red, chain=chain)
         model_bwd(p, g, source, mask, tidx, fw.sv_e, fw.sv_d, fw.dec, None, None, dims, base, scaler_zeros, red, dd=dd, chain=chain)
diff --git a/gpt-st_amd/ops.py b/gpt-st_amd/ops.py
--- a/gpt-st_amd/ops.py
+++ b/gpt-st_amd/ops.py
@@ -220,6 +220,23 @@
     return dS, dW, db, ns
 
 
+class LowRankH1(NamedTuple):
+    source: Any
+    uc: Any
+
+
+def apply_wgrad_guide(dOut, x, W, BT, N):
+    _chk(dOut, x.source, x.uc, W)
+    C = dOut.shape[-1]
+    ns = _C.lib().value("gptst_apply_wgrad_nsplit", MODE_TIME, BT, N)
+    dS = torch.empty_like(dOut)
+    dW = torch.empty(ns * BT, C * C, device=dOut.device, dtype=torch.float32)
+    db = torch.empty(ns * BT, C, device=dOut.device, dtype=torch.float32)
+    _call("gptst_apply_wgrad_guide", _p(dOut), _p(x.source), x.source.shape[-1], _p(x.uc), _p(W), _p(dS), _p(dW), _p(db), BT, N, C,
+          nbytes=_nb(dOut, W, dS, dW))
+    return dS, dW, db, ns
+
+
 def linear_bwd(dY, X, Wp, dOut, out, premul=False):
     _chk(dY, X, Wp, dOut, out)
     rows, C = dY.shape
@@ -274,12 +291,18 @@
     return out
 
 
-def hypertem_fwd(X, G, Wbt, bbt, want_R=True):
+def hypertem_fwd(X, G, Wbt, bbt, want_R=True, guest=None):
     _chk(X, G, Wbt, bbt)
     B, T, N, C = X.shape
     R = torch.empty_like(X) if want_R else None
     out = torch.empty_like(X)
-    _call("gptst_hypertem_fwd", _p(X), _p(G), _p(Wbt), _p(bbt), _p(R), _p(out), B, T, N, C, nbytes=_nb(X, G, Wbt, bbt, R, out))
+    if guest is None:
+        _call("gptst_hypertem_fwd", _p(X), _p(G), _p(Wbt), _p(bbt), _p(R), _p(out), B, T, N, C, nbytes=_nb(X, G, Wbt, bbt, R, out))
+    else:
+        stage, ts, v0, v1, HS, lda, w = guest
+        _chk(*ts)
+        _call("gptst_hypertem_fwd_kl", _p(X), _p(G), _p(Wbt), _p(bbt), _p(R), _p(out), B, T, N, C, stage, _ptrs0(ts), v0, v1, HS, lda, float(w),
+              tag="kl%d" % stage, nbytes=_nb(X, G, Wbt, bbt, R, out))
     return R, out
 
 
@@ -339,7 +362,7 @@
     return h1
 
 
-def guide_head_fwd(source, w1, b1, Wn, bn, Wbt, bbt, W3, b3):
+def guide_head_fwd(source, w1, b1, Wn, bn, Wbt, bbt, W3, b3, want_h1=True, uc=None):
     B, T, N, F = source.shape
     C, J = Wn.shape[-1], W3.shape[0]
     if C != 64 or J > 16:
@@ -347,13 +370,16 @@
     _chk(source, w1, b1, Wn, bn, Wbt, bbt, W3, b3)
     dev = source.device
     f = dict(device=dev, dtype=torch.float32)
-    uc = torch.empty(N, 2 * C, **f)
-    h1, h2 = torch.empty(B * T * N, C, **f), torch.empty(B * T * N, C, **f)
+    if uc is None:
+        uc = torch.empty(N, 2 * C, **f)
+    assert uc.shape == (N, 2 * C)
+    _chk(uc)
+    h1, h2 = torch.empty(B * T * N, C, **f) if want_h1 else None, torch.empty(B * T * N, C, **f)
     prob = torch.empty(B * T * N, J, **f)
     label = torch.empty(B * T * N, device=dev, dtype=torch.int32)
     _call("gptst_guide_head_fwd", _p(source), F, _p(w1), _p(b1), _p(Wn), _p(bn), _p(Wbt), _p(bbt), _p(W3), _p(b3), _p(uc), _p(h1), _p(h2), _p(prob),
           _p(label), B * T, N, C, J, nbytes=_nb(Wbt, h1, h2, prob))
-    return h1, h2, prob, label
+    return h1 if want_h1 else LowRankH1(source, uc), h2, prob, label
 
 
 def guide_in_bwd(dPre, source, w1, b1, Wn):
diff --git a/gpt-st_amd/step.py b/gpt-st_amd/step.py
--- a/gpt-st_amd/step.py
+++ b/gpt-st_amd/step.py
@@ -218,7 +218,7 @@
 
     def _carry_kl(self, sv_g):
         return (self.fused_tails and self.dp is None and not self.global_count_scale and not self.deterministic and not self.safe_mode
-                and not self.always_guide and engine.CTX.NODE_REDUCE is None and engine.kl_carry_ok(self.dims, self.HS, sv_g))
+                and not self.always_guide and engine.CTX.NODE_REDUCE is None and engine.kl_carry_ok(self.dims, self.HS, sv_g, join=self.join_enc_dec))
 
     def _mask_ws(self):
         return self.arena.zeros(ops.mask_ws_floats())
diff --git a/include/gptst_hip.h b/include/gptst_hip.h
--- a/include/gptst_hip.h
+++ b/include/gptst_hip.h
@@ -9,7 +9,7 @@
 #pragma GCC visibility push(default)
 #endif
 
-#define GPTST_ABI_VERSION 16
+#define GPTST_ABI_VERSION 17
 int gptst_abi_version(void);
 int gptst_set_deterministic(int on);
 int gptst_handoff_timeouts(int* out);
@@ -49,6 +49,8 @@
 int gptst_apply_wgrad_nsplit(int mode, int BT, int N);
 int gptst_apply_wgrad(const float* dOut, const float* Y, const float* S, const float* W, float* dS, float* dW, float* colsum, int premul,
                       int mode, int BT, int N, int C, void* stream);
+int gptst_apply_wgrad_guide(const float* dOut, const float* src, int lda, const float* uc, const float* W, float* dS, float* dW, float* colsum,
+                            int BT, int N, int C, void* stream);
 
 int gptst_linear_bwd_nsplit(int rows);
 int gptst_linear_bwd(const float* dY, const float* X, const float* Wp, const float* dOut, const float* out, float* dX, float* dWp, float* dbp,
@@ -70,6 +72,8 @@
                              int B, int T, int N, int C, void* stream);
 int gptst_hypertem_chain_fwd_kl(const float* X, int nstage, const void* Gs, const void* Wbts, const void* bbts, const void* Rs, const void* outs,
                                 int B, int T, int N, int C, int stage, const void* ops, int v0, int v1, int HS, int lda, float w, void* stream);
+int gptst_hypertem_fwd_kl(const float* X, const float* G, const float* Wbt, const float* bbt, float* R_out, float* out, int B, int T, int N, int C,
+                          int stage, const void* ops, int v0, int v1, int HS, int lda, float w, void* stream);
 int gptst_kl_guest_blocks(int stage, int B, int T, int N);
 
 int gptst_encin_ht1_fwd(const float* src, int lda, const float* mask, float fill, const float* w, const float* bi, const float* G,
```

After: 932.5 steps/s, median of 6. No clear change (+0.5%).
